# linusmossberg/monte-carlo-ray-tracer

Hardware: NVIDIA H100
Metric: Mray/s (primary+shadow+bounce) (higher is better)
Workload: dtype f64

## Files before the change

### include/mcrt_abi.h

```cpp
#ifndef MCRT_ABI_H
#define MCRT_ABI_H

#include <stddef.h>
#include <stdint.h>

#ifdef __cplusplus
extern "C" {
#endif

#define MCRT_ABI_VERSION 1

typedef enum mcrt_status {
    MCRT_OK = 0,
    MCRT_ERR_INVALID = -1,
    MCRT_ERR_CUDA = -2,
    MCRT_ERR_NO_SCENE = -3,
    MCRT_ERR_UNSUPPORTED = -4,
    MCRT_ERR_NO_PHOTONS = -5
} mcrt_status;

enum { MCRT_PRIM_TRIANGLE = 0, MCRT_PRIM_SPHERE = 1, MCRT_PRIM_QUADRIC = 2 };

enum { MCRT_INTEGRATOR_PATH = 0, MCRT_INTEGRATOR_PHOTON = 1 };

// ... 257 lines not shown
                                    uint32_t tile, const uint8_t* active_tiles, uint32_t sample_first, uint32_t sample_count,
                                    uint32_t global_seed, int integrator_kind, int precision, double* planes_dev,
                                    uint32_t n_planes, mcrt_stats* stats);

enum {
    MCRT_PM_EMISSION = 0, MCRT_PM_DIRECT = 1, MCRT_PM_CAUSTIC = 2, MCRT_PM_GLOBAL = 3, MCRT_PM_COMPONENT_COUNT = 4
};
int mcrt_render_accumulate_photon_components_dev(mcrt_ctx* ctx, const mcrt_camera* camera, uint32_t y_first, uint32_t y_step,
                                                 uint32_t n_rows, uint32_t tile, const uint8_t* active_tiles,
                                                 uint32_t sample_first, uint32_t sample_count, uint32_t global_seed,
                                                 int integrator_kind, int precision, double* planes_dev, uint32_t n_planes,
                                                 mcrt_stats* stats);

enum {
    MCRT_LPE_SYM_RD = 0, MCRT_LPE_SYM_RS = 1, MCRT_LPE_SYM_RG = 2, MCRT_LPE_SYM_TS = 3, MCRT_LPE_SYM_TG = 4,
    MCRT_LPE_SYM_B = 5, MCRT_LPE_SYM_L = 6, MCRT_LPE_SYM_LABEL0 = 7,
    MCRT_LPE_MAX_EXPRESSIONS = 32, MCRT_LPE_MAX_LABELS = 64, MCRT_LPE_MAX_STATES = 255, MCRT_LPE_DEAD = 255,
    MCRT_LPE_MAX_SYMBOLS = MCRT_LPE_SYM_LABEL0 + MCRT_LPE_MAX_LABELS
};
int mcrt_set_light_path_expressions(mcrt_ctx* ctx, const char* const* exprs, uint32_t n);
int mcrt_render_accumulate_lpe_dev(mcrt_ctx* ctx, const mcrt_camera* camera, uint32_t y_first, uint32_t y_step, uint32_t n_rows,
                                   uint32_t tile, const uint8_t* active_tiles, uint32_t sample_first, uint32_t sample_count,
                                   uint32_t global_seed, int integrator_kind, int precision, double* planes_dev,
                                   uint32_t n_planes, mcrt_stats* stats);
int mcrt_lpe_compile_host(const char* const* exprs, uint32_t n, uint32_t n_groups, uint8_t* next, uint32_t* accept,
                          uint8_t* group_symbol, uint32_t* n_states, uint32_t* n_symbols, char* error, uint32_t error_capacity);
int mcrt_lpe_compile_photon_host(const char* const* exprs, uint32_t n, uint32_t n_groups, uint8_t* rev_next, uint32_t* rev_start,
                                 uint32_t* rev_n_states, uint32_t* join, char* error, uint32_t error_capacity);

int mcrt_render_features_dev(mcrt_ctx* ctx, const mcrt_camera* camera, uint32_t sample_first, uint32_t sample_count,
                             uint32_t global_seed, int precision, double* features_dev, mcrt_stats* stats);

#define MCRT_FEATURES_MAX_SPECULAR_DEPTH 7

int mcrt_render_features_chain_dev(mcrt_ctx* ctx, const mcrt_camera* camera, uint32_t sample_first, uint32_t sample_count,
                                   uint32_t global_seed, int precision, uint32_t specular_depth, double* features_dev,
                                   mcrt_stats* stats);

typedef struct mcrt_denoise_params {
    uint32_t iterations;
    uint32_t _pad;
    double sigma_color, sigma_normal, sigma_depth, sigma_albedo;
} mcrt_denoise_params;

#define MCRT_DENOISE_MAX_ITERATIONS 10
#define MCRT_DENOISE_DEFAULT_ITERATIONS 5
#define MCRT_DENOISE_DEFAULT_SIGMA_COLOR 1.0
#define MCRT_DENOISE_DEFAULT_SIGMA_NORMAL 64.0
#define MCRT_DENOISE_DEFAULT_SIGMA_DEPTH 0.1
#define MCRT_DENOISE_DEFAULT_SIGMA_ALBEDO 0.1

int mcrt_denoise_dev(mcrt_ctx* ctx, const double* a_rgb_dev, const double* a_weight_dev,
                     const double* b_rgb_dev, const double* b_weight_dev, const uint32_t* tile_samples,
                     uint32_t tile, const double* features_dev, uint32_t width, uint32_t height,
                     const mcrt_denoise_params* params, double* out_rgb_dev, double* frame_error);

int mcrt_denoise_planes_dev(mcrt_ctx* ctx, const double* a_rgb_dev, const double* b_rgb_dev,
                            const double* a_planes_dev, const double* b_planes_dev, uint32_t n_planes,
                            const uint32_t* tile_samples, uint32_t tile, const double* features_dev,
                            uint32_t width, uint32_t height, const mcrt_denoise_params* params,
                            double* a_out_planes_dev, double* b_out_planes_dev,
                            double* out_rgb_dev, double* frame_error);

int mcrt_frame_alloc(mcrt_ctx* ctx, uint64_t bytes, void** dev_ptr, unsigned char ipc_handle[64]);
int mcrt_frame_open(mcrt_ctx* ctx, const unsigned char ipc_handle[64], void** dev_ptr);
int mcrt_frame_close(mcrt_ctx* ctx, void* peer_ptr);
int mcrt_frame_free(mcrt_ctx* ctx, void* dev_ptr);

int mcrt_bvh4_host(const mcrt_scene_desc* scene, uint32_t max_leaf, void** handle, const void** nodes128, uint32_t* n_nodes);
void mcrt_bvh4_host_free(void* handle);

int mcrt_fp64_peak(mcrt_ctx* ctx, double* dfma_per_second);

int mcrt_trace_closest(mcrt_ctx* ctx, const mcrt_ray* rays, size_t n, int precision,
                       mcrt_hit* hits, mcrt_stats* stats);

int mcrt_sample_rays(mcrt_ctx* ctx, const mcrt_ray* rays, const uint32_t* pixel,
                     const uint32_t* sample, size_t n, uint32_t global_seed,
                     int integrator_kind, int precision, double* out_rgb, mcrt_stats* stats);

int mcrt_sampler_stream(mcrt_ctx* ctx, const uint32_t* pixel, const uint32_t* sample, size_t n,
                        uint32_t n_shuffles, uint32_t global_seed, uint32_t* out_u32x7);

int mcrt_knn_search(mcrt_ctx* ctx, int which, const double* points_xyz, size_t n,
                    uint32_t* out_index, double* out_dist2, uint32_t* out_count,
                    mcrt_stats* stats);

int mcrt_set_option(mcrt_ctx* ctx, const char* key, double value);

#ifdef __cplusplus
}
#endif
#endif
```

### monte-carlo-ray-tracer_b200/__init__.py

```python
import ctypes as C
import math
import os
import struct

import numpy as np

HERE = os.path.dirname(os.path.abspath(__file__))
LIB_PATH = os.environ.get("MCRT_LIB", os.path.join(HERE, "libmcrt_b200.so"))

INTEGRATOR_PATH, INTEGRATOR_PHOTON = 0, 1
PRECISION_F64, PRECISION_F32 = 0, 1
PRIM_TRIANGLE, PRIM_SPHERE, PRIM_QUADRIC = 0, 1, 2
NO_PRIM = 0xFFFFFFFF

ABI_SYMBOLS = [
    "mcrt_abi_version", "mcrt_init", "mcrt_destroy", "mcrt_last_error", "mcrt_scene_upload",
    "mcrt_photon_upload", "mcrt_photon_emit", "mcrt_photon_download", "mcrt_octree_build",
    "mcrt_octree_free", "mcrt_render_rows", "mcrt_render_rows_dev", "mcrt_render_rows_strided_dev",
    "mcrt_trace_closest",
    "mcrt_sample_rays", "mcrt_sampler_stream", "mcrt_knn_search", "mcrt_set_option", "mcrt_set_film",
    "mcrt_obj_load", "mcrt_obj_free", "mcrt_obj_vertex_normals",
    "mcrt_bvh_build", "mcrt_bvh_free", "mcrt_image_tonemap", "mcrt_image_tonemap_dev",
    "mcrt_render_rows_strided_peers", "mcrt_frame_alloc", "mcrt_frame_open", "mcrt_frame_close", "mcrt_frame_free",
    "mcrt_render_film_sums_strided_dev", "mcrt_film_resolve_dev",
    "mcrt_bvh4_host", "mcrt_bvh4_host_free",
    "mcrt_fp64_peak", "mcrt_photon_emit_total", "mcrt_photon_emit_range", "mcrt_photon_build_dev",
    "mcrt_render_accumulate_dev", "mcrt_progressive_resolve_dev",
    "mcrt_render_accumulate_tiles_dev", "mcrt_progressive_resolve_tiles_dev",
    "mcrt_render_features_dev", "mcrt_denoise_dev", "mcrt_render_features_chain_dev",
    "mcrt_photon_emit_pass", "mcrt_photon_gather_radius", "mcrt_photon_gather_search",
    "mcrt_set_light_groups", "mcrt_render_accumulate_groups_dev", "mcrt_light_groups_combine_dev",
    "mcrt_render_accumulate_aovs_dev", "mcrt_photon_download_lights", "mcrt_render_accumulate_photon_components_dev",
    "mcrt_set_light_path_expressions", "mcrt_render_accumulate_lpe_dev", "mcrt_lpe_compile_host",
    "mcrt_lpe_compile_photon_host", "mcrt_photon_download_lpe_states", "mcrt_denoise_planes_dev",
]

AOV_NAMES = ("background", "emission", "diffuse_direct", "diffuse_indirect", "reflection_direct", "reflection_indirect",
             "transmission_direct", "transmission_indirect")

PHOTON_COMPONENT_NAMES = ("emission", "direct", "caustic", "global")

LPE_SYM_RD, LPE_SYM_RS, LPE_SYM_RG, LPE_SYM_TS, LPE_SYM_TG, LPE_SYM_B, LPE_SYM_L, LPE_SYM_LABEL0 = range(8)
LPE_DEAD, LPE_MAX_STATES, LPE_MAX_SYMBOLS, LPE_MAX_EXPRESSIONS = 255, 255, 71, 32
AOV_LPES = ("CB", "CL", "C<RD>[LB]", "C<RD>.+[LB]", "C[<RS><RG>][LB]", "C[<RS><RG>].+[LB]", "C<T.>[LB]", "C<T.>.+[LB]")


def PM_COMPONENT_LPES(direct_visualization):
    n = "[<RD><RG><TG>]"
    if direct_visualization:
        return ("C<.S>*L", "C.*B", f"C<.S>*{n}<.S>.*L", f"C<.S>*{n}({n}.*)?L")
    return ("C<.S>*L", f"C<.S>*{n}L", f"C<.S>*{n}{{1,2}}<.S>.*L", f"C<.S>*{n}{{2}}({n}.*)?L")


class McrtError(RuntimeError):
    pass


class DenoiseParams(C.Structure):
    _fields_ = [("iterations", C.c_uint32), ("_pad", C.c_uint32), ("sigma_color", C.c_double), ("sigma_normal", C.c_double),
                ("sigma_depth", C.c_double), ("sigma_albedo", C.c_double)]


DENOISE_DEFAULTS = {"iterations": 5, "sigma_color": 1.0, "sigma_normal": 64.0, "sigma_depth": 0.1, "sigma_albedo": 0.1}
FEATURES_MAX_SPECULAR_DEPTH = 7


class MaterialRec(C.Structure):
    _fields_ = [("reflectance", C.c_double * 3), ("specular_reflectance", C.c_double * 3),
                ("transmittance", C.c_double * 3), ("emittance", C.c_double * 3),
                ("roughness", C.c_double), ("specular_roughness", C.c_double), ("ior", C.c_double),
                ("transparency", C.c_double), ("complex_ior_real", C.c_double * 3),
                ("complex_ior_imag", C.c_double * 3), ("A", C.c_double), ("B", C.c_double),
                ("a", C.c_double * 2), ("has_complex_ior", C.c_uint32), ("perfect_mirror", C.c_uint32),
                ("rough", C.c_uint32), ("rough_specular", C.c_uint32), ("opaque", C.c_uint32),
                ("emissive", C.c_uint32), ("dirac_delta", C.c_uint32), ("_pad", C.c_uint32)]


MATERIAL_DTYPE = np.dtype([
    ("reflectance", "<f8", 3), ("specular_reflectance", "<f8", 3), ("transmittance", "<f8", 3),
    ("emittance", "<f8", 3), ("roughness", "<f8"), ("specular_roughness", "<f8"), ("ior", "<f8"),
    ("transparency", "<f8"), ("complex_ior_real", "<f8", 3), ("complex_ior_imag", "<f8", 3),
    ("A", "<f8"), ("B", "<f8"), ("a", "<f8", 2), ("has_complex_ior", "<u4"), ("perfect_mirror", "<u4"),
    ("rough", "<u4"), ("rough_specular", "<u4"), ("opaque", "<u4"), ("emissive", "<u4"),
    ("dirac_delta", "<u4"), ("_pad", "<u4")])
assert MATERIAL_DTYPE.itemsize == C.sizeof(MaterialRec)


class SceneDesc(C.Structure):
    _fields_ = [("abi_version", C.c_uint32), ("n_nodes", C.c_uint32),
                ("node_bounds", C.c_void_p), ("node_first_prim", C.c_void_p),
                ("node_prim_count", C.c_void_p), ("node_next_sibling", C.c_void_p),
                ("n_prims", C.c_uint32),
                ("prim_type", C.c_void_p), ("prim_index", C.c_void_p), ("prim_material", C.c_void_p),
                ("prim_area", C.c_void_p),
                ("n_tris", C.c_uint32),
                ("tri_v0", C.c_void_p), ("tri_v1", C.c_void_p), ("tri_v2", C.c_void_p),
                ("tri_e1", C.c_void_p), ("tri_e2", C.c_void_p), ("tri_normal", C.c_void_p),
                ("tri_vn_index", C.c_void_p),
                ("n_vertex_normals", C.c_uint32), ("vertex_normals", C.c_void_p),
                ("n_spheres", C.c_uint32), ("sphere_origin_radius", C.c_void_p),
                ("n_quadrics", C.c_uint32),
                ("quadric_Q", C.c_void_p), ("quadric_G", C.c_void_p), ("quadric_bounds", C.c_void_p),
                ("n_materials", C.c_uint32), ("materials", C.c_void_p),
# ... 91 lines not shown
        L.mcrt_init.argtypes = [C.c_int, C.POINTER(C.c_void_p)]
        L.mcrt_destroy.argtypes = [C.c_void_p]
        L.mcrt_destroy.restype = None
        L.mcrt_last_error.argtypes = [C.c_void_p]
        L.mcrt_last_error.restype = C.c_char_p
        L.mcrt_scene_upload.argtypes = [C.c_void_p, C.POINTER(SceneDesc), C.POINTER(C.c_uint64)]
        L.mcrt_photon_upload.argtypes = [C.c_void_p, C.POINTER(PhotonMapDesc), C.POINTER(PhotonMapDesc),
                                         C.c_uint32, C.c_uint32, C.POINTER(C.c_uint64)]
        L.mcrt_photon_emit.argtypes = [C.c_void_p, C.POINTER(PhotonEmitParams), C.c_int, C.POINTER(C.c_uint64),
                                       C.POINTER(C.c_uint64), C.POINTER(Stats)]
        L.mcrt_photon_emit_pass.argtypes = [C.c_void_p, C.POINTER(PhotonEmitParams), C.c_int, C.c_uint32, C.POINTER(C.c_uint64),
                                            C.POINTER(C.c_uint64), C.POINTER(Stats)]
        L.mcrt_photon_gather_radius.argtypes = [C.c_void_p, C.c_double, C.c_double]
        L.mcrt_photon_gather_search.argtypes = [C.c_void_p, C.c_int, C.c_void_p, C.c_size_t, C.c_double, C.c_void_p, C.c_void_p,
                                                C.c_void_p, C.POINTER(Stats)]
        L.mcrt_photon_download.argtypes = [C.c_void_p, C.c_int, C.POINTER(PhotonMapDesc)]
        L.mcrt_photon_download_lights.argtypes = [C.c_void_p, C.c_int, C.c_void_p, C.c_uint64]
        L.mcrt_photon_download_lpe_states.argtypes = [C.c_void_p, C.c_int, C.c_void_p, C.c_uint64]
        L.mcrt_octree_build.argtypes = [C.c_void_p, C.c_void_p, C.c_uint64, C.c_uint32, C.c_void_p, C.POINTER(C.c_void_p),
                                        C.POINTER(PhotonMapDesc), C.POINTER(C.c_double)]
        L.mcrt_octree_free.argtypes = [C.c_void_p]
        L.mcrt_octree_free.restype = None
        render_args = [C.c_void_p, C.POINTER(CameraRec), C.c_uint32, C.c_uint32, C.c_uint32, C.c_uint32,
                       C.c_int, C.c_int, C.c_void_p, C.POINTER(Stats)]
        L.mcrt_render_rows.argtypes = render_args
        L.mcrt_render_rows_dev.argtypes = render_args
        L.mcrt_render_rows_strided_dev.argtypes = [C.c_void_p, C.POINTER(CameraRec), C.c_uint32, C.c_uint32, C.c_uint32,
                                                   C.c_uint32, C.c_uint32, C.c_int, C.c_int, C.c_void_p, C.POINTER(Stats)]
        L.mcrt_render_rows_strided_peers.argtypes = [C.c_void_p, C.POINTER(CameraRec), C.c_uint32, C.c_uint32, C.c_uint32, C.c_uint32,
                                                     C.c_uint32, C.c_int, C.c_int, C.c_void_p, C.c_uint32, C.c_int, C.POINTER(Stats)]
        L.mcrt_frame_alloc.argtypes = [C.c_void_p, C.c_uint64, C.POINTER(C.c_void_p), C.c_void_p]
        L.mcrt_frame_open.argtypes = [C.c_void_p, C.c_void_p, C.POINTER(C.c_void_p)]
        L.mcrt_frame_close.argtypes = [C.c_void_p, C.c_void_p]
        L.mcrt_frame_free.argtypes = [C.c_void_p, C.c_void_p]
        L.mcrt_fp64_peak.argtypes = [C.c_void_p, C.POINTER(C.c_double)]
        L.mcrt_bvh4_host.argtypes = [C.POINTER(SceneDesc), C.c_uint32, C.POINTER(C.c_void_p), C.POINTER(C.c_void_p), C.POINTER(C.c_uint32)]
        L.mcrt_bvh4_host_free.argtypes = [C.c_void_p]
        L.mcrt_bvh4_host_free.restype = None
        L.mcrt_render_film_sums_strided_dev.argtypes = [C.c_void_p, C.POINTER(CameraRec), C.c_uint32, C.c_uint32, C.c_uint32, C.c_uint32,
                                                        C.c_uint32, C.c_int, C.c_int, C.c_void_p, C.c_void_p, C.POINTER(Stats)]
        L.mcrt_film_resolve_dev.argtypes = [C.c_void_p, C.c_void_p, C.c_void_p, C.c_uint64, C.c_void_p]
        L.mcrt_render_accumulate_dev.argtypes = [C.c_void_p, C.POINTER(CameraRec), C.c_uint32, C.c_uint32, C.c_uint32, C.c_uint32,
                                                 C.c_uint32, C.c_uint32, C.c_int, C.c_int, C.c_void_p, C.c_void_p, C.POINTER(Stats)]
        L.mcrt_progressive_resolve_dev.argtypes = [C.c_void_p, C.c_void_p, C.c_void_p, C.c_uint64, C.c_void_p, C.c_void_p, C.c_uint64,
                                                   C.c_uint32, C.c_uint32, C.c_uint32, C.c_void_p, C.c_void_p, C.POINTER(C.c_double)]
        L.mcrt_render_accumulate_tiles_dev.argtypes = [C.c_void_p, C.POINTER(CameraRec), C.c_uint32, C.c_uint32, C.c_uint32, C.c_uint32,
                                                       C.c_void_p, C.c_uint32, C.c_uint32, C.c_uint32, C.c_int, C.c_int, C.c_void_p,
                                                       C.c_void_p, C.POINTER(Stats)]
        L.mcrt_progressive_resolve_tiles_dev.argtypes = [C.c_void_p, C.c_void_p, C.c_void_p, C.c_void_p, C.c_void_p, C.c_void_p,
                                                         C.c_uint32, C.c_uint32, C.c_uint32, C.c_void_p, C.c_void_p, C.c_void_p,
                                                         C.POINTER(C.c_double)]
        L.mcrt_set_light_groups.argtypes = [C.c_void_p, C.c_void_p, C.c_uint32, C.c_uint32]
        L.mcrt_render_accumulate_groups_dev.argtypes = [C.c_void_p, C.POINTER(CameraRec), C.c_uint32, C.c_uint32, C.c_uint32, C.c_uint32,
                                                        C.c_void_p, C.c_uint32, C.c_uint32, C.c_uint32, C.c_int, C.c_int, C.c_void_p,
                                                        C.c_uint32, C.POINTER(Stats)]
        L.mcrt_render_accumulate_aovs_dev.argtypes = L.mcrt_render_accumulate_groups_dev.argtypes
        L.mcrt_render_accumulate_photon_components_dev.argtypes = L.mcrt_render_accumulate_groups_dev.argtypes
        L.mcrt_set_light_path_expressions.argtypes = [C.c_void_p, C.c_void_p, C.c_uint32]
        L.mcrt_render_accumulate_lpe_dev.argtypes = L.mcrt_render_accumulate_groups_dev.argtypes
        L.mcrt_lpe_compile_host.argtypes = [C.c_void_p, C.c_uint32, C.c_uint32, C.c_void_p, C.c_void_p, C.c_void_p,
                                            C.POINTER(C.c_uint32), C.POINTER(C.c_uint32), C.c_char_p, C.c_uint32]
        L.mcrt_lpe_compile_photon_host.argtypes = [C.c_void_p, C.c_uint32, C.c_uint32, C.c_void_p, C.POINTER(C.c_uint32),
                                                   C.POINTER(C.c_uint32), C.c_void_p, C.c_char_p, C.c_uint32]
        L.mcrt_light_groups_combine_dev.argtypes = [C.c_void_p, C.c_void_p, C.c_uint32, C.c_uint64, C.c_void_p, C.c_void_p]
        L.mcrt_render_features_dev.argtypes = [C.c_void_p, C.POINTER(CameraRec), C.c_uint32, C.c_uint32, C.c_uint32, C.c_int,
                                               C.c_void_p, C.POINTER(Stats)]
        L.mcrt_render_features_chain_dev.argtypes = [C.c_void_p, C.POINTER(CameraRec), C.c_uint32, C.c_uint32, C.c_uint32, C.c_int,
                                                     C.c_uint32, C.c_void_p, C.POINTER(Stats)]
        L.mcrt_denoise_dev.argtypes = [C.c_void_p, C.c_void_p, C.c_void_p, C.c_void_p, C.c_void_p, C.c_void_p, C.c_uint32,
                                       C.c_void_p, C.c_uint32, C.c_uint32, C.POINTER(DenoiseParams), C.c_void_p,
                                       C.POINTER(C.c_double)]
        L.mcrt_denoise_planes_dev.argtypes = [C.c_void_p, C.c_void_p, C.c_void_p, C.c_void_p, C.c_void_p, C.c_uint32, C.c_void_p,
                                              C.c_uint32, C.c_void_p, C.c_uint32, C.c_uint32, C.POINTER(DenoiseParams), C.c_void_p,
                                              C.c_void_p, C.c_void_p, C.POINTER(C.c_double)]
        L.mcrt_photon_emit_total.argtypes = [C.c_void_p, C.POINTER(PhotonEmitParams), C.POINTER(C.c_uint64)]
        L.mcrt_photon_emit_range.argtypes = [C.c_void_p, C.POINTER(PhotonEmitParams), C.c_int, C.c_uint64, C.c_uint64, C.POINTER(C.c_void_p),
                                             C.POINTER(C.c_uint64), C.POINTER(C.c_void_p), C.POINTER(C.c_uint64), C.POINTER(Stats)]
        L.mcrt_photon_build_dev.argtypes = [C.c_void_p, C.POINTER(PhotonEmitParams), C.c_void_p, C.c_uint64, C.c_void_p, C.c_uint64,
                                            C.POINTER(C.c_double)]
        L.mcrt_trace_closest.argtypes = [C.c_void_p, C.c_void_p, C.c_size_t, C.c_int, C.c_void_p, C.POINTER(Stats)]
        L.mcrt_sample_rays.argtypes = [C.c_void_p, C.c_void_p, C.c_void_p, C.c_void_p, C.c_size_t, C.c_uint32,
                                       C.c_int, C.c_int, C.c_void_p, C.POINTER(Stats)]
        L.mcrt_sampler_stream.argtypes = [C.c_void_p, C.c_void_p, C.c_void_p, C.c_size_t, C.c_uint32, C.c_uint32, C.c_void_p]
        L.mcrt_knn_search.argtypes = [C.c_void_p, C.c_int, C.c_void_p, C.c_size_t, C.c_void_p, C.c_void_p,
                                      C.c_void_p, C.POINTER(Stats)]
        L.mcrt_set_option.argtypes = [C.c_void_p, C.c_char_p, C.c_double]
        L.mcrt_set_film.argtypes = [C.c_void_p, C.POINTER(FilmRec)]
        L.mcrt_bvh_build.argtypes = [C.c_void_p, C.c_void_p, C.c_uint32, C.c_void_p, C.c_int, C.c_int,
                                     C.POINTER(C.c_void_p), C.POINTER(BvhDesc), C.POINTER(C.c_double)]
        L.mcrt_bvh_free.argtypes = [C.c_void_p]
        L.mcrt_bvh_free.restype = None
        L.mcrt_obj_load.argtypes = [C.c_char_p, C.c_int, C.POINTER(C.c_void_p), C.POINTER(ObjMeshRec), C.c_char_p, C.c_size_t]
        L.mcrt_obj_free.argtypes = [C.c_void_p]
        L.mcrt_obj_free.restype = None
        L.mcrt_obj_vertex_normals.argtypes = [C.c_void_p, C.c_uint64, C.c_void_p, C.c_uint64, C.c_int, C.c_void_p]
        tm_args = [C.c_void_p, C.c_void_p, C.c_uint32, C.c_uint32, C.POINTER(ImageParams), C.c_void_p,
                   C.POINTER(C.c_double), C.POINTER(C.c_double)]
        L.mcrt_image_tonemap.argtypes = tm_args
        L.mcrt_image_tonemap_dev.argtypes = tm_args
        if L.mcrt_abi_version() != 1:
            raise McrtError("libmcrt_b200.so ABI version mismatch")
        _lib = L
    return _lib


def _ptr(a):
    return a.ctypes.data_as(C.c_void_p) if a is not None and a.size else None


_PACK_DTYPES = {0: np.uint8, 1: np.uint32, 2: np.int32, 3: np.uint64, 4: np.float32, 5: np.float64}


def read_pack(path):
    if path.endswith(".xz"):
        import lzma
        with lzma.open(path, "rb") as f:
            blob = f.read()
    else:
        with open(path, "rb") as f:
            blob = f.read()
    if blob[:8] != b"MCRTPK01":
        raise McrtError(f"{path}: not a scene pack")
    n, = struct.unpack_from("<I", blob, 8)
    out = {}
    for i in range(n):
        name, dtype, elem_size, count, offset = struct.unpack_from("<32sIIQQ", blob, 16 + 56 * i)
        name = name.split(b"\0")[0].decode()
        if dtype == 6:
            if name != "materials" or elem_size != MATERIAL_DTYPE.itemsize:
                raise McrtError(f"{path}: unexpected struct entry {name}")
            arr = np.frombuffer(blob, dtype=MATERIAL_DTYPE, count=count, offset=offset)
        else:
            arr = np.frombuffer(blob, dtype=_PACK_DTYPES[dtype], count=count, offset=offset)
        out[name] = arr.copy()
    return out


class Scene:

    _ARRAYS = ["node_bounds", "node_first_prim", "node_prim_count", "node_next_sibling", "prim_type",
               "prim_index", "prim_material", "prim_area", "tri_v0", "tri_v1", "tri_v2", "tri_e1", "tri_e2",
               "tri_normal", "tri_vn_index", "vertex_normals", "sphere_origin_radius", "quadric_Q",
               "quadric_G", "quadric_bounds", "materials", "light_prim", "light_cdf"]

    def __init__(self, arrays):
        self.a = {k: np.ascontiguousarray(arrays[k]) for k in self._ARRAYS}
        self.ior = float(np.asarray(arrays["scene_ior"]).reshape(-1)[0])
        self.extra = {k: v for k, v in arrays.items() if k not in self._ARRAYS}

    @classmethod
    def from_pack(cls, path):
        return cls(read_pack(path))

    @property
    def n_prims(self):
        return int(self.a["prim_type"].size)

    @property
    def n_nodes(self):
        return int(self.a["node_first_prim"].size)

    @property
    def n_lights(self):
        return int(self.a["light_prim"].size)

    def desc(self):
# ... 358 lines not shown
        return self.last_stats

    def denoise_dev(self, a_rgb_ptr, a_weight_ptr, b_rgb_ptr, b_weight_ptr, tile_samples, tile, features_ptr, width, height,
                    out_ptr, params=None):
        def p(x):
            return C.c_void_p(x) if x else None
        counts = np.ascontiguousarray(tile_samples, dtype=np.uint32)
        if counts.shape != tile_grid(height, width, tile) + (2,):
            raise McrtError(f"tile_samples has shape {counts.shape}, expected {tile_grid(height, width, tile) + (2,)}")
        err = C.c_double()
        self._check(lib().mcrt_denoise_dev(self.ctx, p(a_rgb_ptr), p(a_weight_ptr), p(b_rgb_ptr), p(b_weight_ptr),
                                           counts.ctypes.data_as(C.c_void_p), tile, p(features_ptr), width, height,
                                           C.byref(params) if params is not None else None, p(out_ptr), C.byref(err)))
        return err.value

    def denoise_planes_dev(self, a_rgb_ptr, b_rgb_ptr, a_planes_ptr, b_planes_ptr, n_planes, tile_samples, tile, features_ptr,
                           width, height, a_out_ptr, b_out_ptr, params=None, out_ptr=None):
        def p(x):
            return C.c_void_p(x) if x else None
        counts = np.ascontiguousarray(tile_samples, dtype=np.uint32)
        if counts.shape != tile_grid(height, width, tile) + (2,):
            raise McrtError(f"tile_samples has shape {counts.shape}, expected {tile_grid(height, width, tile) + (2,)}")
        err = C.c_double()
        self._check(lib().mcrt_denoise_planes_dev(self.ctx, p(a_rgb_ptr), p(b_rgb_ptr), p(a_planes_ptr), p(b_planes_ptr), n_planes,
                                                  counts.ctypes.data_as(C.c_void_p), tile, p(features_ptr), width, height,
                                                  C.byref(params) if params is not None else None, p(a_out_ptr), p(b_out_ptr),
                                                  p(out_ptr), C.byref(err) if out_ptr else None))
        return err.value if out_ptr else None

    def frame_alloc(self, nbytes):
        ptr = C.c_void_p(); h = (C.c_ubyte * 64)()
        self._check(lib().mcrt_frame_alloc(self.ctx, nbytes, C.byref(ptr), h))
        return ptr.value, bytes(h)

    def frame_open(self, handle):
        ptr = C.c_void_p(); h = (C.c_ubyte * 64)(*handle)
        self._check(lib().mcrt_frame_open(self.ctx, h, C.byref(ptr)))
        return ptr.value

    def frame_close(self, ptr):
        self._check(lib().mcrt_frame_close(self.ctx, C.c_void_p(ptr)))

    def frame_free(self, ptr):
        self._check(lib().mcrt_frame_free(self.ctx, C.c_void_p(ptr)))

    def fp64_peak(self):
        v = C.c_double()
        self._check(lib().mcrt_fp64_peak(self.ctx, C.byref(v)))
        return v.value

    def render_rows_strided_dev(self, camera, out_dev_ptr, y_first, y_step, n_rows, sqrtspp=None, precision=None):
        self.set_film(camera)
        st = Stats()
        self._check(lib().mcrt_render_rows_strided_dev(self.ctx, C.byref(camera.rec), y_first, y_step, n_rows,
                                                       camera.sqrtspp if sqrtspp is None else sqrtspp,
                                                       self.global_seed, self.kind,
                                                       self.precision if precision is None else precision,
                                                       C.c_void_p(out_dev_ptr), C.byref(st)))
        self.last_stats = st.as_dict()
        return self.last_stats

    def tonemap(self, rgb, image=None):
        params = image if isinstance(image, ImageParams) else ImageParams.from_json(image or {})
        rgb = np.ascontiguousarray(rgb, dtype=np.float64)
        h, w = rgb.shape[:2]
        out = np.zeros((h, w, 3), dtype=np.uint8)
        e, g = C.c_double(), C.c_double()
        self._check(lib().mcrt_image_tonemap(self.ctx, _ptr(rgb), w, h, C.byref(params), _ptr(out), C.byref(e), C.byref(g)))
        return out, e.value, g.value

    def tonemap_dev(self, rgb_dev_ptr, out_dev_ptr, width, height, image=None):
        params = image if isinstance(image, ImageParams) else ImageParams.from_json(image or {})
        e, g = C.c_double(), C.c_double()
        self._check(lib().mcrt_image_tonemap_dev(self.ctx, C.c_void_p(rgb_dev_ptr), width, height, C.byref(params),
                                                 C.c_void_p(out_dev_ptr), C.byref(e), C.byref(g)))
        return e.value, g.value

    def sampler_stream(self, pixel, sample, n_shuffles):
        pixel = np.ascontiguousarray(pixel, dtype=np.uint32)
        sample = np.ascontiguousarray(sample, dtype=np.uint32)
        out = np.zeros((len(pixel), 7), dtype=np.uint32)
        self._check(lib().mcrt_sampler_stream(self.ctx, _ptr(pixel), _ptr(sample), len(pixel), n_shuffles,
                                              self.global_seed, _ptr(out)))
        return out


class PathTracer(Integrator):
    kind = INTEGRATOR_PATH


class PhotonMapper(Integrator):
    kind = INTEGRATOR_PHOTON

    def __init__(self, scene, device=0, precision=PRECISION_F64, global_seed=0x12345678, photon_maps=None, emit=None):
        super().__init__(scene, device, precision, global_seed)
        if emit is not None:
            self.emit(**emit)
            return
        maps = photon_maps or scene.photon_maps()
        if maps is None:
            raise McrtError("PhotonMapper needs photon maps (scene pack exported with photon_map=True) or emit=...")
        self._maps = maps
        self.upload_photons()

    @property
    def has_photon_lights(self):
        return getattr(self, "_photon_lights", False)

    @property
    def has_photon_lpe_states(self):
        key = getattr(self, "_photon_lpe_key", None)
        return key is not None and getattr(self, "_emitted", None) is not None and key == getattr(self, "_lpe_key", None)

    def photon_lpe_states(self, which):
        out = np.zeros(self.n_photons[which], np.uint32)
        self._check(lib().mcrt_photon_download_lpe_states(self.ctx, int(which), _ptr(out), out.size))
        return out

    def emit_again(self):
        if getattr(self, "_emit_args", None) is None:
            raise McrtError("the photon maps did not come from emit() / emit_pass()")
        return self.emit_pass(*self._emit_args)

    def photon_lights(self, which):
        if not self.has_photon_lights:
            raise McrtError("the photon maps carry no light index: only the maps of emit() / emit_pass() do")
        out = np.zeros(self.n_photons[which], np.uint32)
        self._check(lib().mcrt_photon_download_lights(self.ctx, int(which), _ptr(out), out.size))
        return out

    def set_light_groups(self, ids, n_groups=None):
        if not self.has_photon_lights:
            raise McrtError("the photon mapper has no light groups with these maps: their photons carry no light index "
                            "(only the maps of emit() / emit_pass() do)")
        return super().set_light_groups(ids, n_groups)

    def render_accumulate_aovs_dev(self, *args, **kwargs):
        raise McrtError("the photon mapper has no light-path AOVs")

    def render_accumulate_components_dev(self, camera, planes_ptr, sample_first, sample_count, tile=0, active=None,
                                         y_first=0, y_step=1, n_rows=None, precision=None):
        return self._render_accumulate_planes(lib().mcrt_render_accumulate_photon_components_dev, camera, planes_ptr,
                                              len(PHOTON_COMPONENT_NAMES), sample_first, sample_count, tile, active, y_first,
                                              y_step, n_rows, precision)

    def _emit_params(self, emissions, caustic_factor, max_photons_per_octree_leaf, k_nearest_photons, direct_visualization, scene_bounds):
        p = PhotonEmitParams()
        p.emissions = int(emissions); p.caustic_factor = float(caustic_factor)
        p.max_photons_per_octree_leaf = int(max_photons_per_octree_leaf); p.k_nearest_photons = int(k_nearest_photons)
        p.direct_visualization = int(bool(direct_visualization)); p.global_seed = self.global_seed
        if scene_bounds is not None:
            b = scene_bounds
        elif self.scene.a["node_bounds"].size >= 6:
            b = self.scene.a["node_bounds"][:6]
        elif "scene_bounds" in self.scene.extra:
            b = self.scene.extra["scene_bounds"]
        else:
            raise McrtError("the scene has no BVH and no scene bounds: pass scene_bounds")
        for i in range(6):
            p.scene_bounds[i] = float(b[i])
        return p

    def emit_sharded(self, rank, world, emissions, caustic_factor, max_photons_per_octree_leaf=200, k_nearest_photons=50,
                     direct_visualization=False, scene_bounds=None, precision=None):
        import torch
        from . import distributed as mdist
# ... 837 lines not shown
```

### monte-carlo-ray-tracer_b200/csrc/abi.cu

```cuda
#include <algorithm>
#include <cmath>
#include <cstdio>
#include <cstdlib>
#include <cstring>
#include <string>
#include <vector>

#include "mcrt_abi.h"
#include "launch.h"
#include "bvh_build.h"
#include "image.h"
#include "denoise.h"
#include "lpe.h"

using namespace mcrt;

static const int MCRT_INTERNAL_EMIT = 100;

#define CK(call)                                                                              \
    do {                                                                                      \
        cudaError_t e_ = (call);                                                              \
        if (e_ != cudaSuccess)                                                                \
        {                                                                                     \
            ctx->error = std::string(#call) + ": " + cudaGetErrorString(e_);                  \
// ... 472 lines not shown
            const Pending pn = queue[q];
            const uint32_t self = (uint32_t)out.size();
            out.emplace_back();
            out[pn.parent].child[pn.slot] = self;
            expand(pn.item, kids);
            too_big = emit(kids, self) != 0;
        }
        if (too_big) out.clear();
        return MCRT_OK;
    }

    template <class R>
    int uploadArrays(mcrt_ctx* ctx, const mcrt_scene_desc& s, SceneArrays<R>& a, uint64_t& bytes)
    {
        DeviceScene<R>& d = a.dev;
        int rc;
        if ((rc = devUpload(ctx, ctx->scene_allocs, &d.wide, a.wide, bytes))) return rc;
        if ((rc = devUpload(ctx, ctx->scene_allocs, &d.geom, a.geom, bytes))) return rc;
        if ((rc = devUpload(ctx, ctx->scene_allocs, &d.shade, a.shade, bytes))) return rc;
        if ((rc = devUpload(ctx, ctx->scene_allocs, &d.vnormals, a.vnormals, bytes))) return rc;
        if ((rc = devUpload(ctx, ctx->scene_allocs, &d.quadrics, a.quadrics, bytes))) return rc;
        if ((rc = devUpload(ctx, ctx->scene_allocs, &d.materials, a.materials, bytes))) return rc;
        if ((rc = devUpload(ctx, ctx->scene_allocs, &d.lights, a.lights, bytes))) return rc;
        {
            std::vector<uint32_t> combos;
            std::vector<uint8_t> cls(s.n_prims ? s.n_prims : 1, 1);
            for (uint32_t i = 0; i < s.n_prims; i++)
            {
                const uint32_t combo = (a.materials[a.shade[i].material].flags << 1) | (a.shade[i].vn_index >= 0 ? 1u : 0u);
                size_t k = 0;
                while (k < combos.size() && combos[k] != combo) k++;
                if (k == combos.size()) combos.push_back(combo);
                cls[i] = (uint8_t)(1u + (k < SHADE_CLASS_BINS - 1u ? k : SHADE_CLASS_BINS - 2u));
            }
            if ((rc = devUpload(ctx, ctx->scene_allocs, &d.shade_class, cls, bytes))) return rc;
        }
        d.n_nodes = s.n_nodes; d.n_prims = s.n_prims; d.n_lights = s.n_lights;
        d.prims_class = PRIMS_TRI;
        for (uint32_t i = 0; i < s.n_prims; i++)
        {
            if (s.prim_type[i] == MCRT_PRIM_SPHERE && d.prims_class == PRIMS_TRI) d.prims_class = PRIMS_TRI_SPHERE;
            else if (s.prim_type[i] != MCRT_PRIM_TRIANGLE && s.prim_type[i] != MCRT_PRIM_SPHERE) { d.prims_class = PRIMS_ALL; break; }
        }
        d.material_flags_any = 0;
        for (const auto& m : a.materials) d.material_flags_any |= m.flags;
        d.scene_ior = (R)s.scene_ior;
        d.scene_scale = (R)ctx->scene_scale;
        return MCRT_OK;
    }

    template <class R>
    int ensureWave(mcrt_ctx* ctx, WaveBuffers<R>& w, std::vector<void*>& track)
    {
        if (w.capacity == ctx->pool_paths) return MCRT_OK;
        freeAll(track);
        w.capacity = 0;
        const size_t n = ctx->pool_paths;
        int rc;
        for (int b = 0; b < 2; b++)
        {
            if ((rc = devAlloc(ctx, track, &w.buf[b].ray_o, n))) return rc;
            if ((rc = devAlloc(ctx, track, &w.buf[b].ray_d, n))) return rc;
            if ((rc = devAlloc(ctx, track, &w.buf[b].thr, n))) return rc;
            if ((rc = devAlloc(ctx, track, &w.buf[b].iors_a, n))) return rc;
            if ((rc = devAlloc(ctx, track, &w.buf[b].iors_b, n))) return rc;
            if ((rc = devAlloc(ctx, track, &w.buf[b].meta, n))) return rc;
            if ((rc = devAlloc(ctx, track, &w.buf[b].meta2, n))) return rc;
        }
        if ((rc = devAlloc(ctx, track, &w.shadow, n))) return rc;
        if ((rc = devAlloc(ctx, track, &w.hits, n))) return rc;
        w.capacity = ctx->pool_paths;
        return MCRT_OK;
    }

    int ensureSort(mcrt_ctx* ctx)
    {
        if (ctx->sort_capacity == ctx->pool_paths) return MCRT_OK;
        freeAll(ctx->sort_allocs);
        ctx->sort_capacity = 0;
        const size_t n = ctx->pool_paths;
        int rc;
        RaySort& r = ctx->sort;
        for (int b = 0; b < 2; b++)
        {
            if ((rc = devAlloc(ctx, ctx->sort_allocs, &r.path_key[b], n))) return rc;
            if ((rc = devAlloc(ctx, ctx->sort_allocs, &r.path_rank[b], n))) return rc;
        }
        if ((rc = devAlloc(ctx, ctx->sort_allocs, &r.path_order, n))) return rc;
        if ((rc = devAlloc(ctx, ctx->sort_allocs, &r.shadow_key, n))) return rc;
        if ((rc = devAlloc(ctx, ctx->sort_allocs, &r.shadow_rank, n))) return rc;
        if ((rc = devAlloc(ctx, ctx->sort_allocs, &r.shadow_order, n))) return rc;
        if ((rc = devAlloc(ctx, ctx->sort_allocs, &r.shade_key, n))) return rc;
        if ((rc = devAlloc(ctx, ctx->sort_allocs, &r.shade_rank, n))) return rc;
        if ((rc = devAlloc(ctx, ctx->sort_allocs, &r.shade_order, n))) return rc;
        if ((rc = devAlloc(ctx, ctx->sort_allocs, &r.hist_shade, (size_t)SORT_BINS))) return rc;
        if ((rc = devAlloc(ctx, ctx->sort_allocs, &r.hist_path, (size_t)SORT_BINS))) return rc;
        if ((rc = devAlloc(ctx, ctx->sort_allocs, &r.hist_shadow, (size_t)SORT_BINS))) return rc;
        if ((rc = devAlloc(ctx, ctx->sort_allocs, &r.bin_start, (size_t)SORT_BINS))) return rc;
        if ((rc = devAlloc(ctx, ctx->sort_allocs, &r.block_offset, (size_t)2 * SORT_SCAN_BLOCKS))) return rc;
        if ((rc = devAlloc(ctx, ctx->sort_allocs, &r.done_counter, (size_t)1))) return rc;
        CK(cudaMemset(r.done_counter, 0, sizeof(uint32_t)));
        ctx->sort_capacity = ctx->pool_paths;
        return MCRT_OK;
    }

    int ensureFilm(mcrt_ctx* ctx, size_t values)
    {
        if (ctx->film_values >= values && ctx->d_film) return MCRT_OK;
        if (ctx->d_film) cudaFree(ctx->d_film);
        ctx->d_film = nullptr; ctx->film_values = 0;
        CK(cudaMalloc((void**)&ctx->d_film, values * sizeof(double)));
        ctx->film_values = values;
        return MCRT_OK;
    }

    template <class R> DeviceScene<R>& sceneOf(mcrt_ctx* ctx);
    template <> DeviceScene<double>& sceneOf<double>(mcrt_ctx* ctx) { return ctx->scene64; }
    template <> DeviceScene<float>& sceneOf<float>(mcrt_ctx* ctx) { return ctx->scene32; }
    template <class R> WaveBuffers<R>& waveOf(mcrt_ctx* ctx);
    template <> WaveBuffers<double>& waveOf<double>(mcrt_ctx* ctx) { return ctx->wave64; }
    template <> WaveBuffers<float>& waveOf<float>(mcrt_ctx* ctx) { return ctx->wave32; }
    template <class R> std::vector<void*>& waveAllocsOf(mcrt_ctx* ctx);
    template <> std::vector<void*>& waveAllocsOf<double>(mcrt_ctx* ctx) { return ctx->wave_allocs64; }
    template <> std::vector<void*>& waveAllocsOf<float>(mcrt_ctx* ctx) { return ctx->wave_allocs32; }

    void fillStats(mcrt_stats* st, const Counters& c, uint64_t iterations, uint64_t launches, double ms)
    {
        if (!st) return;
        std::memset(st, 0, sizeof(*st));
        st->paths = c.paths;
        st->extension_rays = c.extension_rays;
        st->shadow_rays = c.shadow_rays;
        st->box_tests = c.box_tests;
        st->prim_tests = c.prim_tests;
        st->knn_queries = c.knn_queries;
        st->wavefront_iterations = iterations;
        st->kernel_launches = launches;
        st->ior_stack_overflows = c.ior_stack_overflows;
        st->max_depth = c.max_depth;
        st->gpu_ms_total = ms;
        st->shadow_box_tests = c.shadow_box_tests;
        st->shadow_prim_tests = c.shadow_prim_tests;
        st->extend_work_sum = c.work_sum;
        st->extend_work_warpmax = c.work_warpmax;
        st->replayed_rays = c.replayed_rays;
    }

    template <class R> DeviceCamera<R> deviceCamera(const mcrt_camera& cam)
    {
        DeviceCamera<R> c;
        std::memset(&c, 0, sizeof(c));
        c.eye = v3<R>(cam.eye); c.forward = v3<R>(cam.forward);
        c.left = v3<R>(cam.left); c.up = v3<R>(cam.up);
        c.focal_length = (R)cam.focal_length; c.sensor_width = (R)cam.sensor_width;
        c.aperture_radius = (R)cam.aperture_radius; c.focus_distance = (R)cam.focus_distance;
        c.width = cam.width; c.height = cam.height; c.thin_lens = cam.thin_lens;
        return c;
    }

    template <class R> R rayEps(const mcrt_ctx* ctx)
    {
        return Mode<R>::parity ? (R)1e-9 : (R)(ctx->ray_eps_scale * ctx->scene_scale);
    }

    struct FilmSums
    {
        double* rgb;
        double* wsum;
        uint32_t n_planes = 0;
        bool aovs = false;
        bool lpe = false;
    };

    template <class R>
    int runWavefront(mcrt_ctx* ctx, const mcrt_camera* cam, uint32_t row_first, uint32_t row_step, uint32_t n_pixels, uint32_t spp,
                     uint64_t total_work, uint32_t global_seed, int integrator, const double* d_user_rays,
                     const uint32_t* d_user_pixel, const uint32_t* d_user_sample, size_t film_pixels,
                     double film_weight, double* out_dev, mcrt_stats* stats, uint32_t sample_first = 0,
                     const FilmSums* accum = nullptr, const uint32_t* d_pixel_list = nullptr)
    {
        if (!ctx->has_scene) { ctx->error = "no scene uploaded"; return MCRT_ERR_NO_SCENE; }
        if (integrator == MCRT_INTEGRATOR_PHOTON && !ctx->has_photons)
        {
// ... 83 lines not shown
        if (ctx->sort_rays)
        {
            if ((rc = ensureSort(ctx))) return rc;
            p.sort = ctx->sort;
            p.sort.shade_sorted = ctx->sort_shade ? 1u : 0u;
            if (!ctx->sort_shade_class || integrator == MCRT_INTERNAL_EMIT) p.sort.shade_order = nullptr;
            {
                const uint32_t n_prims = sceneOf<R>(ctx).n_prims;
                const double cells = (double)(1u << (3 * SORT_ORIGIN_BITS));
                const bool use_prim = (ctx->sort_prim_key < 0 ? n_prims >= 4096u : ctx->sort_prim_key != 0) && (double)n_prims >= cells;
                p.sort.prim_scale = use_prim ? (uint32_t)(cells * 4294967296.0 / (double)n_prims * 0.999999) : 0u;
            }
            for (int k = 0; k < 3; k++)
            {
                const double ext = ctx->scene_bmax[k] - ctx->scene_bmin[k];
                p.sort.key_min[k] = (float)ctx->scene_bmin[k];
                p.sort.key_scale[k] = ext > 0.0 ? (float)((double)(1u << SORT_ORIGIN_BITS) / ext) : 0.0f;
            }
        }

        const bool emitting = integrator == MCRT_INTERNAL_EMIT;
        if (emitting)
        {
            p.emit.emit_offsets = ctx->d_emit_offsets;
            p.emit.photon_flux = static_cast<const V4<R>*>(ctx->d_emit_flux);
            p.emit.photons[0] = ctx->d_emit_photons[0]; p.emit.photons[1] = ctx->d_emit_photons[1];
            p.emit.lights[0] = ctx->d_emit_lights[0]; p.emit.lights[1] = ctx->d_emit_lights[1];
            p.emit.capacity[0] = ctx->emit_capacity[0]; p.emit.capacity[1] = ctx->emit_capacity[1];
            p.emit.non_caustic_reject = (R)ctx->emit_non_caustic_reject;
            p.emit.pass = ctx->emit_pass;
            if (ctx->d_emit_lpe_states[0])
            {
                p.emit.lpe_states[0] = ctx->d_emit_lpe_states[0]; p.emit.lpe_states[1] = ctx->d_emit_lpe_states[1];
                p.emit.lpe_rev_next = ctx->d_lpe_rev_next;
                p.emit.lpe_rev_start = ctx->lpe_rev_start;
                p.lpe_light_symbol = ctx->d_lpe_light_symbol;
                p.lpe_symbols = ctx->lpe_symbols;
            }
        }
        if (integrator == MCRT_INTEGRATOR_PHOTON)
        {
            p.pm.map[0] = ctx->photon_map[0]; p.pm.map[1] = ctx->photon_map[1];
            p.pm.queries = knn_queue;
            p.pm.k_nearest = ctx->k_nearest;
            p.pm.direct_visualization = ctx->direct_visualization;
            p.pm.query_capacity = knn_capacity;
            p.pm.gather_r2[0] = ctx->gather_r2[0]; p.pm.gather_r2[1] = ctx->gather_r2[1];
            if (ctx->photon_lights) { p.pm.lights[0] = ctx->built_dev[0].lights; p.pm.lights[1] = ctx->built_dev[1].lights; }
            if (accum && accum->lpe)
            {
                p.pm.lpe_states[0] = ctx->built_dev[0].lpe_states; p.pm.lpe_states[1] = ctx->built_dev[1].lpe_states;
                p.pm.lpe_join = ctx->d_lpe_join;
                p.pm.lpe_join_any = ctx->d_lpe_join_any;
                p.pm.lpe_rev_states = ctx->lpe_rev_states;
            }
        }

        Counters init;
        std::memset(&init, 0, sizeof(init));
        init.total_work = total_work;
        if (sample_first)
        {
            init.next_work = (uint64_t)sample_first * n_pixels;
            init.total_work = init.next_work + total_work;
        }
        if (integrator == MCRT_INTERNAL_EMIT) { init.next_work = ctx->emit_work_first; init.total_work = ctx->emit_work_first + total_work; }
        ctx->h_counters[0] = init;
        CK(cudaEventRecord(ctx->ev_start, s));
        CK(cudaMemcpyAsync(ctx->d_counters, &ctx->h_counters[0], sizeof(Counters), cudaMemcpyHostToDevice, s));
        if (!accum)
        {
            CK(cudaMemsetAsync(ctx->d_film, 0, film_pixels * 3 * sizeof(double), s));
            if (filtered) CK(cudaMemsetAsync(ctx->d_film_wsum, 0, film_pixels * sizeof(double), s));
        }
        const bool sorting = ctx->sort_rays != 0;
        if (sorting)
        {
            CK(cudaMemsetAsync(p.sort.hist_path, 0, SORT_BINS * sizeof(uint32_t), s));
            CK(cudaMemsetAsync(p.sort.hist_shadow, 0, SORT_BINS * sizeof(uint32_t), s));
            CK(cudaMemsetAsync(ctx->sort.hist_shade, 0, SORT_BINS * sizeof(uint32_t), s));
        }
        auto sortPaths = [&](int buffer)
        {
            launchSortScan(p.sort.hist_path, p.sort, s);
            launchSortScatter(p.sort.path_key[buffer], p.sort.path_rank[buffer], p.sort, p.sort.path_order,
                              &ctx->d_counters->n_cur, grid, s);
        };

        uint64_t launches = 0, iterations = 0;

        if (emitting) Launch<R>::emitGenerate(p, 0, grid, s);
        else Launch<R>::generate(p, 0, grid, s);
        launchAdvance(ctx->d_counters, s);
        launches += 2;
        if (sorting) { sortPaths(0); launches += 2; }

        int pending[2] = { 0, 0 };
        int slot = 0;
        bool done = false;
        while (!done)
        {
            for (int k = 0; k < ctx->poll_interval; k++)
            {
                const int cur = (int)(iterations & 1u);
                cudaEvent_t* ev = nullptr;
                if (ctx->stage_timing)
                {
                    while (ctx->stage_events.size() < 6 * (iterations + 1))
                    {
                        cudaEvent_t e;
                        CK(cudaEventCreate(&e));
                        ctx->stage_events.push_back(e);
                    }
                    ev = &ctx->stage_events[6 * iterations];
                    cudaEventRecord(ev[0], s);
                }
                Launch<R>::extend(p, cur, grid, s);
                if (ev) cudaEventRecord(ev[1], s);
                if (p.sort.shade_order)
                {
                    Launch<R>::shadeKey(p, grid, s);
                    launchSortScan(p.sort.hist_shade, p.sort, s);
                    launchSortScatter(p.sort.shade_key, p.sort.shade_rank, p.sort, p.sort.shade_order, &ctx->d_counters->n_cur, grid, s);
                    launches += 3;
                }
                if (emitting)
                {
                    Launch<R>::emitShade(p, cur, grid, s);
                }
                else if (integrator == MCRT_INTEGRATOR_PHOTON)
                {
                    Launch<R>::shadePhoton(p, cur, grid, s);
                    if (ev) cudaEventRecord(ev[5], s);
                    Launch<R>::knn(p, grid, s);
                    launches += 1;
                }
                else
                {
                    Launch<R>::shade(p, cur, grid, s);
                }
                if (ev) cudaEventRecord(ev[2], s);
                if (!emitting)
                {
                    if (sorting)
                    {
                        launchSortScan(p.sort.hist_shadow, p.sort, s);
                        launchSortScatter(p.sort.shadow_key, p.sort.shadow_rank, p.sort, p.sort.shadow_order,
                                          &ctx->d_counters->n_shadow, grid, s);
                        launches += 2;
                    }
                    Launch<R>::shadow(p, grid, s);
                }
                if (ev) cudaEventRecord(ev[3], s);
                if (emitting) Launch<R>::emitGenerate(p, cur ^ 1, grid, s);
                else Launch<R>::generate(p, cur ^ 1, grid, s);
                launchAdvance(ctx->d_counters, s);
                if (sorting) { sortPaths(cur ^ 1); launches += 2; }
                if (ev) cudaEventRecord(ev[4], s);
                launches += 5;
                iterations++;
            }
            CK(cudaMemcpyAsync(&ctx->h_counters[slot], ctx->d_counters, sizeof(Counters), cudaMemcpyDeviceToHost, s));
            CK(cudaEventRecord(ctx->ev_poll[slot], s));
            pending[slot] = 1;
            const int other = slot ^ 1;
            if (pending[other])
            {
                CK(cudaEventSynchronize(ctx->ev_poll[other]));
                const Counters& c = ctx->h_counters[other];
                if (c.n_cur == 0 && c.next_work >= c.total_work) done = true;
                pending[other] = 0;
            }
            slot = other;
        }

        if (!emitting && !accum)
        {
            if (filtered) launchResolveFilmWeighted(ctx->d_film, ctx->d_film_wsum, out_dev, film_pixels, grid, s);
            else if (ctx->peer_out.n_frames) launchResolveFilmPeers(ctx->d_film, ctx->peer_out, film_pixels * 3, film_weight, grid, s);
            else launchResolveFilm(ctx->d_film, out_dev, film_pixels * 3, film_weight, grid, s);
            launches += 1;
        }
        CK(cudaEventRecord(ctx->ev_stop, s));
        CK(cudaMemcpyAsync(&ctx->h_counters[0], ctx->d_counters, sizeof(Counters), cudaMemcpyDeviceToHost, s));
        CK(cudaStreamSynchronize(s));
        CK(cudaGetLastError());
        float ms = 0.f;
        CK(cudaEventElapsedTime(&ms, ctx->ev_start, ctx->ev_stop));
        const Counters& c = ctx->h_counters[0];
        fillStats(stats, c, iterations, launches, ms);
        if (stats)
        {
            stats->extend_launches = iterations;
            stats->shadow_launches = iterations;
            if (ctx->stage_timing)
            {
                for (uint64_t it = 0; it < iterations; it++)
                {
                    cudaEvent_t* ev = &ctx->stage_events[6 * it];
                    if (integrator == MCRT_INTEGRATOR_PHOTON) { float tk = 0; cudaEventElapsedTime(&tk, ev[5], ev[2]); stats->gpu_ms_knn += tk; }
                    float t01 = 0, t12 = 0, t23 = 0, t34 = 0;
                    cudaEventElapsedTime(&t01, ev[0], ev[1]); cudaEventElapsedTime(&t12, ev[1], ev[2]);
                    cudaEventElapsedTime(&t23, ev[2], ev[3]); cudaEventElapsedTime(&t34, ev[3], ev[4]);
                    stats->gpu_ms_extend += t01; stats->gpu_ms_shade += t12;
                    stats->gpu_ms_shadow += t23; stats->gpu_ms_generate += t34;
                }
            }
        }
        if (c.traversal_overflow)
        {
            ctx->error = "traversal stack/heap overflow: result would differ from the reference";
            return MCRT_ERR_UNSUPPORTED;
        }
        if (c.ior_stack_overflows)
        {
            ctx->error = "more than 8 nested dielectric media on a path (refraction-history stack overflow): result would differ from the reference";
            return MCRT_ERR_UNSUPPORTED;
        }
        if (emitting && c.photon_overflow)
        {
            ctx->error = "photon arrays overflowed";
            return MCRT_ERR_UNSUPPORTED;
        }
        return MCRT_OK;
    }

    int renderDispatch(mcrt_ctx* ctx, const mcrt_camera* camera, uint32_t y_first, uint32_t y_step, uint32_t n_rows,
                       uint32_t sample_first, uint64_t spp, uint32_t global_seed, int integrator_kind, int precision,
                       double* out_dev, mcrt_stats* stats, const FilmSums* accum = nullptr,
                       const uint32_t* d_pixel_list = nullptr, uint32_t n_list = 0)
    {
        if (!camera || n_rows == 0 || y_step == 0 || spp == 0 || camera->width == 0 ||
            (uint64_t)y_first + (uint64_t)(n_rows - 1) * y_step >= camera->height)
        {
            ctx->error = "mcrt_render_rows: invalid camera / row range / sample count";
            return MCRT_ERR_INVALID;
        }
        if ((uint64_t)sample_first + spp > 0x100000000ull)
        {
            ctx->error = "sample range beyond 2^32 samples per pixel";
// ... 1641 lines not shown
        rc = runWavefront<float>(ctx, nullptr, 0, 1, 0, 1, n, global_seed, integrator_kind, d_rays, d_pixel, d_sample, n, 1.0, d_out, stats);
    else { ctx->error = "unknown precision"; rc = MCRT_ERR_INVALID; }
    if (rc == MCRT_OK && cudaMemcpy(out_rgb, d_out, n * 3 * sizeof(double), cudaMemcpyDeviceToHost) != cudaSuccess)
    { ctx->error = "copy back failed"; rc = MCRT_ERR_CUDA; }
    cleanup();
    return rc;
}

int mcrt_trace_closest(mcrt_ctx* ctx, const mcrt_ray* rays, size_t n, int precision, mcrt_hit* hits, mcrt_stats* stats)
{
    if (!ctx) return MCRT_ERR_INVALID;
    if (n == 0) return MCRT_OK;
    if (!rays || !hits) { ctx->error = "mcrt_trace_closest: null buffer"; return MCRT_ERR_INVALID; }
    if (!ctx->has_scene) { ctx->error = "no scene uploaded"; return MCRT_ERR_NO_SCENE; }
    CK(cudaSetDevice(ctx->device));
    double* d_rays = nullptr; double* d_tuv = nullptr; uint32_t* d_prim = nullptr;
    auto cleanup = [&]() { cudaFree(d_rays); cudaFree(d_tuv); cudaFree(d_prim); };
    if (cudaMalloc((void**)&d_rays, n * 6 * sizeof(double)) != cudaSuccess || cudaMalloc((void**)&d_tuv, n * 3 * sizeof(double)) != cudaSuccess ||
        cudaMalloc((void**)&d_prim, n * 4) != cudaSuccess)
    { cleanup(); ctx->error = "cudaMalloc failed"; return MCRT_ERR_CUDA; }
    cudaStream_t s = ctx->stream;
    cudaMemcpyAsync(d_rays, rays, n * 6 * sizeof(double), cudaMemcpyHostToDevice, s);
    cudaMemsetAsync(ctx->d_counters, 0, sizeof(Counters), s);
    const int grid = ctx->sm_count * ctx->blocks_per_sm;
    cudaEventRecord(ctx->ev_start, s);
    if (precision == MCRT_PRECISION_F64)
    {
        DeviceScene<double> sc = ctx->scene64;
        if (ctx->exact_traversal) sc.bvh4 = nullptr;
        Launch<double>::traceUser(sc, d_rays, n, d_tuv, d_prim, ctx->d_counters, grid, s);
    }
    else if (precision == MCRT_PRECISION_F32) Launch<float>::traceUser(ctx->scene32, d_rays, n, d_tuv, d_prim, ctx->d_counters, grid, s);
    else { cleanup(); ctx->error = "unknown precision"; return MCRT_ERR_INVALID; }
    cudaEventRecord(ctx->ev_stop, s);
    std::vector<double> tuv(n * 3);
    std::vector<uint32_t> prim(n);
    cudaMemcpyAsync(tuv.data(), d_tuv, n * 3 * sizeof(double), cudaMemcpyDeviceToHost, s);
    cudaMemcpyAsync(prim.data(), d_prim, n * 4, cudaMemcpyDeviceToHost, s);
    cudaMemcpyAsync(&ctx->h_counters[0], ctx->d_counters, sizeof(Counters), cudaMemcpyDeviceToHost, s);
    cudaError_t e = cudaStreamSynchronize(s);
    if (e == cudaSuccess) e = cudaGetLastError();
    cleanup();
    if (e != cudaSuccess) { ctx->error = cudaGetErrorString(e); return MCRT_ERR_CUDA; }
    float ms = 0.f;
    cudaEventElapsedTime(&ms, ctx->ev_start, ctx->ev_stop);
    fillStats(stats, ctx->h_counters[0], 0, 1, ms);
    for (size_t i = 0; i < n; i++)
    {
        const bool interp = prim[i] != NO_PRIM && ctx->prim_interpolates[prim[i]];
        hits[i].t = tuv[3 * i];
        hits[i].u = interp ? tuv[3 * i + 1] : 0.0;
        hits[i].v = interp ? tuv[3 * i + 2] : 0.0;
        hits[i].prim = prim[i];
        hits[i].interpolate = interp ? 1u : 0u;
    }
    if (ctx->h_counters[0].traversal_overflow) { ctx->error = "traversal stack/heap overflow"; return MCRT_ERR_UNSUPPORTED; }
    return MCRT_OK;
}

int mcrt_sampler_stream(mcrt_ctx* ctx, const uint32_t* pixel, const uint32_t* sample, size_t n, uint32_t n_shuffles,
                        uint32_t global_seed, uint32_t* out_u32x7)
{
    if (!ctx) return MCRT_ERR_INVALID;
    if (n == 0) return MCRT_OK;
    if (!pixel || !sample || !out_u32x7) { ctx->error = "mcrt_sampler_stream: null buffer"; return MCRT_ERR_INVALID; }
    CK(cudaSetDevice(ctx->device));
    uint32_t* d_pixel = nullptr; uint32_t* d_sample = nullptr; uint32_t* d_out = nullptr;
    auto cleanup = [&]() { cudaFree(d_pixel); cudaFree(d_sample); cudaFree(d_out); };
    if (cudaMalloc((void**)&d_pixel, n * 4) != cudaSuccess || cudaMalloc((void**)&d_sample, n * 4) != cudaSuccess ||
        cudaMalloc((void**)&d_out, n * 28) != cudaSuccess)
    { cleanup(); ctx->error = "cudaMalloc failed"; return MCRT_ERR_CUDA; }
    cudaStream_t s = ctx->stream;
    cudaMemcpyAsync(d_pixel, pixel, n * 4, cudaMemcpyHostToDevice, s);
    cudaMemcpyAsync(d_sample, sample, n * 4, cudaMemcpyHostToDevice, s);
    launchSamplerStream(d_pixel, d_sample, n, n_shuffles, global_seed, d_out, s);
    cudaMemcpyAsync(out_u32x7, d_out, n * 28, cudaMemcpyDeviceToHost, s);
    cudaError_t e = cudaStreamSynchronize(s);
    if (e == cudaSuccess) e = cudaGetLastError();
    cleanup();
    if (e != cudaSuccess) { ctx->error = cudaGetErrorString(e); return MCRT_ERR_CUDA; }
    return MCRT_OK;
}

int mcrt_knn_search(mcrt_ctx* ctx, int which, const double* points_xyz, size_t n, uint32_t* out_index, double* out_dist2,
                    uint32_t* out_count, mcrt_stats* stats)
{
    if (!ctx) return MCRT_ERR_INVALID;
    if (n == 0) return MCRT_OK;
    if (!points_xyz || !out_index || !out_dist2 || !out_count || (which != 0 && which != 1))
    { ctx->error = "mcrt_knn_search: invalid arguments"; return MCRT_ERR_INVALID; }
    if (!ctx->has_photons) { ctx->error = "no photon maps uploaded"; return MCRT_ERR_NO_PHOTONS; }
    CK(cudaSetDevice(ctx->device));
    const uint32_t k = ctx->k_nearest;
    double* d_pts = nullptr; uint32_t* d_idx = nullptr; double* d_d2 = nullptr; uint32_t* d_cnt = nullptr; uint32_t* d_flag = nullptr;
    auto cleanup = [&]() { cudaFree(d_pts); cudaFree(d_idx); cudaFree(d_d2); cudaFree(d_cnt); cudaFree(d_flag); };
    if (cudaMalloc((void**)&d_pts, n * 24) != cudaSuccess || cudaMalloc((void**)&d_idx, n * k * 4) != cudaSuccess ||
        cudaMalloc((void**)&d_d2, n * k * 8) != cudaSuccess || cudaMalloc((void**)&d_cnt, n * 4) != cudaSuccess ||
        cudaMalloc((void**)&d_flag, 4) != cudaSuccess)
    { cleanup(); ctx->error = "cudaMalloc failed"; return MCRT_ERR_CUDA; }
    cudaStream_t s = ctx->stream;
    cudaMemcpyAsync(d_pts, points_xyz, n * 24, cudaMemcpyHostToDevice, s);
    cudaMemsetAsync(d_flag, 0, 4, s);
    cudaEventRecord(ctx->ev_start, s);
    launchKnnUser(ctx->photon_map[which], k, d_pts, n, d_idx, d_d2, d_cnt, d_flag, ctx->sm_count * ctx->blocks_per_sm, s);
    cudaEventRecord(ctx->ev_stop, s);
    uint32_t flag = 0;
    cudaMemcpyAsync(out_index, d_idx, n * k * 4, cudaMemcpyDeviceToHost, s);
    cudaMemcpyAsync(out_dist2, d_d2, n * k * 8, cudaMemcpyDeviceToHost, s);
    cudaMemcpyAsync(out_count, d_cnt, n * 4, cudaMemcpyDeviceToHost, s);
    cudaMemcpyAsync(&flag, d_flag, 4, cudaMemcpyDeviceToHost, s);
    cudaError_t e = cudaStreamSynchronize(s);
    if (e == cudaSuccess) e = cudaGetLastError();
    cleanup();
    if (e != cudaSuccess) { ctx->error = cudaGetErrorString(e); return MCRT_ERR_CUDA; }
    float ms = 0.f;
    cudaEventElapsedTime(&ms, ctx->ev_start, ctx->ev_stop);
    if (stats) { std::memset(stats, 0, sizeof(*stats)); stats->knn_queries = n; stats->gpu_ms_total = ms; stats->gpu_ms_knn = ms; }
    if (flag) { ctx->error = "k-NN frontier overflow"; return MCRT_ERR_UNSUPPORTED; }
    return MCRT_OK;
}

int mcrt_photon_gather_radius(mcrt_ctx* ctx, double r_caustic, double r_global)
{
    if (!ctx) return MCRT_ERR_INVALID;
    if (r_caustic == 0.0 && r_global == 0.0) { ctx->gather_r2[0] = ctx->gather_r2[1] = 0.0; return MCRT_OK; }
    const double r[2] = { r_caustic, r_global };
    for (int w = 0; w < 2; w++)
        if (!(r[w] > 0.0) || !std::isfinite(r[w] * r[w]))
        { ctx->error = "mcrt_photon_gather_radius: radii must be (0, 0) or two positive finite numbers"; return MCRT_ERR_INVALID; }
    ctx->gather_r2[0] = r_caustic * r_caustic; ctx->gather_r2[1] = r_global * r_global;
    return MCRT_OK;
}

int mcrt_photon_gather_search(mcrt_ctx* ctx, int which, const double* points_xyz, size_t n, double radius, uint32_t* out_count,
                              double* out_flux_sum, double* out_cone_sum, mcrt_stats* stats)
{
    if (!ctx) return MCRT_ERR_INVALID;
    if ((which != 0 && which != 1) || !(radius > 0.0) || !std::isfinite(radius * radius))
    { ctx->error = "mcrt_photon_gather_search: invalid arguments"; return MCRT_ERR_INVALID; }
    if (n == 0) return MCRT_OK;
    if (!points_xyz || !out_count || !out_flux_sum || !out_cone_sum) { ctx->error = "mcrt_photon_gather_search: null buffer"; return MCRT_ERR_INVALID; }
    if (!ctx->has_photons) { ctx->error = "no photon maps uploaded"; return MCRT_ERR_NO_PHOTONS; }
    CK(cudaSetDevice(ctx->device));
    double* d_pts = nullptr; uint32_t* d_cnt = nullptr; double* d_flux = nullptr; double* d_cone = nullptr; uint32_t* d_flag = nullptr;
    auto cleanup = [&]() { cudaFree(d_pts); cudaFree(d_cnt); cudaFree(d_flux); cudaFree(d_cone); cudaFree(d_flag); };
    if (cudaMalloc((void**)&d_pts, n * 24) != cudaSuccess || cudaMalloc((void**)&d_cnt, n * 4) != cudaSuccess ||
        cudaMalloc((void**)&d_flux, n * 24) != cudaSuccess || cudaMalloc((void**)&d_cone, n * 24) != cudaSuccess ||
        cudaMalloc((void**)&d_flag, 4) != cudaSuccess)
    { cleanup(); ctx->error = "cudaMalloc failed"; return MCRT_ERR_CUDA; }
    cudaStream_t s = ctx->stream;
    cudaMemcpyAsync(d_pts, points_xyz, n * 24, cudaMemcpyHostToDevice, s);
    cudaMemsetAsync(d_flag, 0, 4, s);
    cudaEventRecord(ctx->ev_start, s);
    launchGatherUser(ctx->photon_map[which], d_pts, n, radius * radius, d_cnt, d_flux, d_cone, d_flag, ctx->sm_count * ctx->blocks_per_sm, s);
    cudaEventRecord(ctx->ev_stop, s);
    uint32_t flag = 0;
    cudaMemcpyAsync(out_count, d_cnt, n * 4, cudaMemcpyDeviceToHost, s);
    cudaMemcpyAsync(out_flux_sum, d_flux, n * 24, cudaMemcpyDeviceToHost, s);
    cudaMemcpyAsync(out_cone_sum, d_cone, n * 24, cudaMemcpyDeviceToHost, s);
    cudaMemcpyAsync(&flag, d_flag, 4, cudaMemcpyDeviceToHost, s);
    cudaError_t e = cudaStreamSynchronize(s);
    if (e == cudaSuccess) e = cudaGetLastError();
    cleanup();
    if (e != cudaSuccess) { ctx->error = cudaGetErrorString(e); return MCRT_ERR_CUDA; }
    float ms = 0.f;
    cudaEventElapsedTime(&ms, ctx->ev_start, ctx->ev_stop);
// ... 7 lines not shown
```

### monte-carlo-ray-tracer_b200/csrc/integrator.cuh

```cuda
#pragma once

#include "bsdf.cuh"
#include "intersect.cuh"
#include "bvh4.cuh"
#include "photon.cuh"
#include "film.cuh"
#include "mcrt_abi.h"

#ifndef MCRT_TRACE_MINBLOCKS_F64
#define MCRT_TRACE_MINBLOCKS_F64 2
#endif
#ifndef MCRT_TRACE_MINBLOCKS_F32
#define MCRT_TRACE_MINBLOCKS_F32 4
#endif
#ifndef MCRT_TRACE_MINBLOCKS_F64_PRUNED
#define MCRT_TRACE_MINBLOCKS_F64_PRUNED 4
#endif
#ifndef MCRT_TRACE_MINBLOCKS_FAST
#define MCRT_TRACE_MINBLOCKS_FAST 2
#endif
#ifndef MCRT_TRACE_MINBLOCKS_DYN
#define MCRT_TRACE_MINBLOCKS_DYN 4
#endif
#ifndef MCRT_KNN_MINBLOCKS
#define MCRT_KNN_MINBLOCKS 8
#endif
#ifndef MCRT_GATHER_MINBLOCKS
#define MCRT_GATHER_MINBLOCKS 3
#endif
#ifndef MCRT_SHADE_MINBLOCKS
#define MCRT_SHADE_MINBLOCKS 3
#endif
#ifndef MCRT_SHADE_MINBLOCKS_LITE
#define MCRT_SHADE_MINBLOCKS_LITE 3
#endif
#ifndef MCRT_SORT_ORIGIN_BITS
#define MCRT_SORT_ORIGIN_BITS 4
#endif
#ifndef MCRT_SORT_DIR_Q
#define MCRT_SORT_DIR_Q 1
#endif

namespace mcrt
{
    constexpr int IOR_STACK_CAPACITY = 8;

    struct Counters
    {
        uint32_t n_cur, n_next, n_shadow, n_gen;
        unsigned long long next_work, total_work;
        unsigned long long paths, extension_rays, shadow_rays, box_tests, prim_tests, knn_queries;
        unsigned long long shadow_box_tests, shadow_prim_tests;
        unsigned long long ior_stack_overflows;
        unsigned long long replayed_rays;
        uint32_t fetch_extend, fetch_shadow;
        uint32_t traversal_overflow, max_depth;
        uint32_t n_knn, _pad;
        unsigned long long work_sum, work_warpmax;
        unsigned long long n_photons[2];
        uint32_t photon_overflow, _pad2;
    };

    template <class R> struct PathBuffer
    {
        V4<R>* ray_o;
        V4<R>* ray_d;
        V4<R>* thr;
        V4<R>* iors_a;
        V4<R>* iors_b;
        uint4* meta;
        uint4* meta2;
    };

    template <class R> struct alignas(16 * sizeof(R)) ShadowRecord
    {
        V4<R> o;
        V4<R> d;
        uint4 meta;
        V4<R> k;
    };
    static_assert(sizeof(ShadowRecord<double>) == 128 && sizeof(ShadowRecord<float>) == 64, "one shadow record per line");
    static_assert(offsetof(ShadowRecord<double>, k) == 96, "the float64 padding is the 16-byte chunk 5 (k_shade writes it)");

    constexpr uint32_t SORT_ORIGIN_BITS = MCRT_SORT_ORIGIN_BITS;
    constexpr uint32_t SORT_DIR_Q = MCRT_SORT_DIR_Q;
    constexpr uint32_t SORT_DIR_BITS = 3 + 2 * SORT_DIR_Q;
    constexpr uint32_t SORT_KEY_BITS = 3 * SORT_ORIGIN_BITS + SORT_DIR_BITS;
    constexpr uint32_t SORT_BINS = 1u << SORT_KEY_BITS;

    struct RaySort
    {
        uint32_t* path_key[2];
        uint32_t* path_rank[2];
        uint32_t* path_order;
        uint32_t* shadow_key;
        uint32_t* shadow_rank;
        uint32_t* shadow_order;
        uint32_t* hist_path;
        uint32_t* hist_shadow;
        uint32_t* bin_start;
        uint32_t* block_offset;
        uint32_t* done_counter;
        uint32_t shade_sorted;
        uint32_t* shade_key;
        uint32_t* shade_rank;
        uint32_t* shade_order;
        uint32_t* hist_shade;
        uint32_t prim_scale;
        float key_min[3], key_scale[3];
    };

    MCRT_D uint32_t spreadBits3(uint32_t v)
    {
        v = (v | (v << 16)) & 0x030000FFu;
        v = (v | (v << 8)) & 0x0300F00Fu;
        v = (v | (v << 4)) & 0x030C30C3u;
        v = (v | (v << 2)) & 0x09249249u;
        return v;
    }

    template <class R>
    MCRT_D uint32_t rayKey(const RaySort& rs, const V3<R>& o, const V3<R>& d, uint32_t src_prim)
    {
        uint32_t cell;
        if (rs.prim_scale && src_prim != NO_PRIM)
        {
            cell = (uint32_t)(((unsigned long long)src_prim * rs.prim_scale) >> 32);
        }
        else
        {
            constexpr float CELLS = (float)(1u << SORT_ORIGIN_BITS);
            float cx = ((float)o.x - rs.key_min[0]) * rs.key_scale[0];
            float cy = ((float)o.y - rs.key_min[1]) * rs.key_scale[1];
            float cz = ((float)o.z - rs.key_min[2]) * rs.key_scale[2];
            uint32_t ix = (uint32_t)fminf(fmaxf(cx, 0.0f), CELLS - 1.0f);
            uint32_t iy = (uint32_t)fminf(fmaxf(cy, 0.0f), CELLS - 1.0f);
            uint32_t iz = (uint32_t)fminf(fmaxf(cz, 0.0f), CELLS - 1.0f);
            cell = spreadBits3(ix) | (spreadBits3(iy) << 1) | (spreadBits3(iz) << 2);
        }
        float dx = (float)d.x, dy = (float)d.y, dz = (float)d.z;
        float ax = fabsf(dx), ay = fabsf(dy), az = fabsf(dz);
        uint32_t face; float u, v, m;
        if (ax >= ay && ax >= az) { face = dx < 0.0f ? 1u : 0u; u = dy; v = dz; m = ax; }
        else if (ay >= az)        { face = dy < 0.0f ? 3u : 2u; u = dx; v = dz; m = ay; }
        else                      { face = dz < 0.0f ? 5u : 4u; u = dx; v = dy; m = az; }
        constexpr float Q = (float)(1u << SORT_DIR_Q);
        float inv = m > 0.0f ? 0.5f * Q / m : 0.0f;
        uint32_t qu = (uint32_t)fminf(fmaxf(u * inv + 0.5f * Q, 0.0f), Q - 1.0f);
        uint32_t qv = (uint32_t)fminf(fmaxf(v * inv + 0.5f * Q, 0.0f), Q - 1.0f);
        uint32_t dir = (face << (2 * SORT_DIR_Q)) | (qu << SORT_DIR_Q) | qv;
        return (dir << (3 * SORT_ORIGIN_BITS)) | cell;
    }

    MCRT_D uint32_t sortRank(uint32_t* hist, uint32_t key, bool pred)
    {
        const unsigned active = __ballot_sync(0xFFFFFFFFu, pred);
        uint32_t rank = 0;
        if (pred)
        {
            const unsigned peers = __match_any_sync(active, key);
            const unsigned lane = threadIdx.x & 31u;
            const int leader = __ffs(peers) - 1;
            uint32_t base = 0;
            if ((int)lane == leader) base = atomicAdd(&hist[key], (uint32_t)__popc(peers));
            base = __shfl_sync(peers, base, leader);
            rank = base + __popc(peers & ((1u << lane) - 1u));
        }
        return rank;
    }

    template <class R> struct EmitParams
    {
        const unsigned long long* emit_offsets;
        const V4<R>* photon_flux;
        float4* photons[2];
        uint32_t* lights[2];
        unsigned long long capacity[2];
        R non_caustic_reject;
        uint32_t pass;
        const uint8_t* lpe_rev_next;
        uint32_t lpe_rev_start;
        uint32_t* lpe_states[2];
    };

    template <class R> struct WaveParams
    {
        DeviceScene<R> scene;
        DeviceCamera<R> camera;
        PathBuffer<R> buf[2];
        ShadowRecord<R>* shadow;
        V4<R>* hits;
        Counters* counters;
        double* film;
        const double* user_rays;
        const uint32_t* user_pixel;
        const uint32_t* user_sample;
        const uint32_t* pixel_list;
        uint32_t capacity;
        uint32_t global_seed;
        uint32_t spp;
        uint32_t row_first;
        uint32_t row_step;
        uint32_t n_pixels;
        uint32_t integrator;
        R ray_eps;
        PhotonParams<R> pm;
        RaySort sort;
        const uint32_t* sobol_bytes;
        EmitParams<R> emit;
        FilmParams filmp;
        const uint32_t* group_of_light;
        size_t plane_values;
        uint32_t n_planes;
        uint32_t aovs;
        const uint8_t* lpe_next;
        const uint32_t* lpe_accept;
        const uint8_t* lpe_light_symbol;
        uint32_t lpe_symbols;
    };

    template <class R> struct Mode;
    template <> struct Mode<double> { static constexpr bool parity = true; static constexpr int trace_minblocks = MCRT_TRACE_MINBLOCKS_F64; static constexpr int trace_minblocks_pruned = MCRT_TRACE_MINBLOCKS_F64_PRUNED; };
    template <> struct Mode<float> { static constexpr bool parity = false; static constexpr int trace_minblocks = MCRT_TRACE_MINBLOCKS_F32; static constexpr int trace_minblocks_pruned = MCRT_TRACE_MINBLOCKS_F32; };

    template <int PRIMS = PRIMS_ALL, bool FAST = false, class R>
    MCRT_D Hit<R> traceClosest(const DeviceScene<R>& sc, const V3<R>& o, const V3<R>& d, uint32_t skip_prim,
                               TraceCounters& cnt, uint32_t& overflow)
    {
        RayQ<R> rq;
        rq.o = o; rq.d = d;
        if constexpr (!(Mode<R>::parity && FAST) || PRIMS == PRIMS_ALL) rq.inv_d = R(1) / d;
        if constexpr (Mode<R>::parity)
        {
            if constexpr (FAST)
            {
                bool ambiguous;
                Hit<R> h = traverseFast<PRIMS>(sc, rq, cnt, ambiguous);
                if (ambiguous)
                {
                    const DeviceScene<R> sc_copy = sc;
                    RayQ<R> rq_copy = rq;
                    rq_copy.inv_d = R(1) / d;
                    Hit<R> h2;
                    traceReferenceOrderOutOfLine<PRIMS>(&sc_copy, &rq_copy, &h2, &cnt.box_tests, &cnt.prim_tests, &overflow);
                    h = h2;
                    cnt.replayed++;
                }
                return h;
            }
            else
            {
// ... 144 lines not shown

    template <class R>
    MCRT_D void cameraRay(const DeviceCamera<R>& c, R scene_ior, uint32_t pixel, const SamplerState& smp,
                          V3<R>& start, V3<R>& direction)
    {
        const uint32_t x = pixel % c.width, y = pixel / c.width;
        R pixel_size = c.sensor_width / R(c.width);
        R half_w = R(c.width) * R(0.5), half_h = R(c.height) * R(0.5);
        R u[2];
        samplerGet<R, DIM_PIXEL, 2>(smp, u);
        R px = R(x) + u[0], py = R(y) + u[1];
        R lx = pixel_size * (half_w - px), ly = pixel_size * (half_h - py);
        direction = normalize(c.forward * c.focal_length + c.left * lx + c.up * ly);
        start = c.eye;
        if (c.thin_lens)
        {
            R ul[2];
            samplerGet<R, DIM_LENS, 2>(smp, ul);
            R azimuth = ul[1] * Consts<R>::TWO_PI;
            R sn, cs;
            msincos(azimuth, &sn, &cs);
            R su = msqrt(ul[0]);
            R ax = (cs * su) * c.aperture_radius, ay = (sn * su) * c.aperture_radius;
            V3<R> focus_point = start + direction * (c.focus_distance / dot(direction, c.forward));
            V3<R> s2 = c.eye + c.left * ax + c.up * ay;
            direction = normalize(focus_point - s2);
            start = s2;
        }
    }

    template <class R, bool FILM, bool LIST>
    __global__ void __launch_bounds__(256) k_generate(WaveParams<R> p, int next)
    {
        Counters* c = p.counters;
        const uint32_t n_next = c->n_next;
        const unsigned long long remaining = c->total_work - c->next_work;
        const uint32_t room = p.capacity - n_next;
        const uint32_t count = remaining < (unsigned long long)room ? (uint32_t)remaining : room;
        if (blockIdx.x == 0 && threadIdx.x == 0) c->n_gen = count;
        const unsigned long long base_work = c->next_work;
        const PathBuffer<R>& out = p.buf[next];

        const uint32_t count_rounded = (count + 31u) & ~31u;
        for (uint32_t j = blockIdx.x * blockDim.x + threadIdx.x; j < count_rounded; j += gridDim.x * blockDim.x)
        {
            const bool valid = j < count;
            uint32_t key = 0;
            const uint32_t slot = n_next + j;
            if (valid)
            {
            const unsigned long long w = base_work + j;
            uint32_t pixel, sample, film_index;
            V3<R> start, direction;
            if (p.user_rays)
            {
                pixel = p.user_pixel[w];
                sample = p.user_sample[w];
                film_index = (uint32_t)w;
                const double* r = p.user_rays + 6 * w;
                start = V3<R>((R)r[0], (R)r[1], (R)r[2]);
                direction = V3<R>((R)r[3], (R)r[4], (R)r[5]);
            }
            else
            {
                uint32_t local = (uint32_t)(w % p.n_pixels);
                if constexpr (LIST) local = p.pixel_list[local];
                sample = (uint32_t)(w / p.n_pixels);
                const uint32_t row = local / p.camera.width, col = local - row * p.camera.width;
                pixel = (p.row_first + row * p.row_step) * p.camera.width + col;
                film_index = local;
                SamplerState smp = SamplerState::make(p.global_seed, pixel, sample, 0u);
                cameraRay(p.camera, p.scene.scene_ior, pixel, smp, start, direction);
                if constexpr (FILM) filmSplatSampleWeight(p.filmp, p.global_seed, pixel, sample);
            }
            stStream(&out.ray_o[slot], V4<R>(start, p.scene.scene_ior));
            stStream(&out.ray_d[slot], V4<R>(direction, R(1)));
            stStream(&out.thr[slot], V4<R>(R(1), R(1), R(1), R(0)));
            stStream(&out.meta[slot], make_uint4(pixel, sample, 0u, 0u));
            stStream(&out.meta2[slot], make_uint4(NO_PRIM, 1u, film_index, NO_PRIM));
            if (p.sort.path_order) key = rayKey(p.sort, start, direction, NO_PRIM);
            }
            if (p.sort.path_order)
            {
                const uint32_t rank = sortRank(p.sort.hist_path, key, valid);
                if (valid) { p.sort.path_key[next][slot] = key; p.sort.path_rank[next][slot] = rank; }
            }
        }
    }

    static __global__ void k_advance(Counters* c)
    {
        c->n_cur = c->n_next + c->n_gen;
        c->next_work += c->n_gen;
        c->paths += c->n_gen;
        c->n_next = 0;
        c->n_gen = 0;
        c->n_shadow = 0;
        c->n_knn = 0;
        c->fetch_extend = 0;
        c->fetch_shadow = 0;
    }

    template <class R, int PRIMS, int FAST>
    __global__ void __launch_bounds__(256, FAST == 2 ? MCRT_TRACE_MINBLOCKS_DYN : (FAST == 1 ? MCRT_TRACE_MINBLOCKS_FAST : (PRIMS == PRIMS_ALL ? Mode<R>::trace_minblocks : Mode<R>::trace_minblocks_pruned))) k_extend(WaveParams<R> p, int cur)
    {
        const uint32_t n = p.counters->n_cur;
        const PathBuffer<R>& in = p.buf[cur];
        TraceCounters cnt = { 0u, 0u, 0u };
        uint32_t overflow = 0;
        unsigned long long rays = 0;
        const uint32_t* order = p.sort.path_order;
        if constexpr (Mode<R>::parity && FAST == 2)
        {
            traceManyFast<PRIMS>(p.scene, n, &p.counters->fetch_extend,
                [&](uint32_t ii, RayQ<R>& r)
                {
                    const uint32_t i = order ? order[ii] : ii;
                    const V4<R> ro = ldStream(&in.ray_o[i]), rd = ldStream(&in.ray_d[i]);
                    r.o = ro.xyz(); r.d = rd.xyz();
                    if constexpr (PRIMS == PRIMS_ALL) r.inv_d = R(1) / r.d;
                    return i;
                },
                [&](uint32_t i, const RayQ<R>&, const Hit<R>& h)
                {
                    stStream(&p.hits[i], V4<R>(h.t, h.u, h.v, h.prim == NO_PRIM ? R(-1) : R(h.prim)));
                    rays++;
                }, cnt, overflow);
            flushStats(p.counters, cnt, rays, false, overflow);
            return;
        }
        for (uint32_t ii = blockIdx.x * blockDim.x + threadIdx.x; ii < n; ii += gridDim.x * blockDim.x)
        {
            const uint32_t i = order ? order[ii] : ii;
            const V4<R> ro = ldStream(&in.ray_o[i]);
            const V4<R> rd = ldStream(&in.ray_d[i]);
            uint32_t skip = NO_PRIM;
            if constexpr (!Mode<R>::parity) skip = in.meta2[i].w;
#ifdef MCRT_TAIL_DIAGNOSTIC
            const uint32_t w0 = cnt.box_tests + cnt.prim_tests;
#endif
            Hit<R> h = traceClosest<PRIMS, FAST != 0>(p.scene, ro.xyz(), rd.xyz(), skip, cnt, overflow);
            stStream(&p.hits[i], V4<R>(h.t, h.u, h.v, h.prim == NO_PRIM ? R(-1) : R(h.prim)));
            rays++;
#ifdef MCRT_TAIL_DIAGNOSTIC
            const uint32_t w = cnt.box_tests + cnt.prim_tests - w0;
            const unsigned am = __activemask();
            const uint32_t wmax = __reduce_max_sync(am, w);
            atomicAdd(&p.counters->work_sum, (unsigned long long)w);
            if ((threadIdx.x & 31u) == (unsigned)(__ffs(am) - 1)) atomicAdd(&p.counters->work_warpmax, 32ull * wmax);
#endif
        }
        flushStats(p.counters, cnt, rays, false, overflow);
    }

    template <class R>
    MCRT_D void sampleLightPoint(const Light<R>& l, R u, R v, V3<R>& pos, V3<R>& normal)
    {
        if (l.type == PRIM_TRIANGLE)
        {
            R su = msqrt(u);
            pos = (R(1) - su) * l.p0 + (R(1) - v) * su * l.p1 + v * su * l.p2;
            normal = l.normal;
        }
        else
        {
            R z = R(1) - R(2) * u;
            R r = msqrt(R(1) - pow2(z));
            R phi = Consts<R>::TWO_PI * v;
// ... 219 lines not shown
                        R cos_light_theta = dot(-s_dir, light_normal);
                        if (cos_light_theta > R(0))
                        {
                            bool ok = true;
                            R cos_theta = dot(s_dir, ia.normal);
                            if (cos_theta <= R(0))
                            {
                                if ((m.flags & MAT_OPAQUE) || cos_theta == R(0)) ok = false;
                                else
                                {
                                    s_start = ia.position - ia.normal * p.ray_eps;
                                    s_dir = normalize(light_pos - s_start);
                                }
                            }
                            if (ok)
                            {
                                V3<R> bsdf_absIdotN; R bsdf_pdf;
                                if (ia.bsdfWorld(bsdf_absIdotN, s_dir, bsdf_pdf))
                                {
                                    want_shadow = true;
                                    sh_o = s_start; sh_d = s_dir;
                                    sh_k = bsdf_absIdotN * L.emittance * throughput;
                                    sh_bsdf_pdf = bsdf_pdf;
                                    sh_area_cos = L.area * cos_light_theta;
                                    sh_select = ls_select;
                                    sh_light = L.prim;
                                    if constexpr (FILM == FILM_MODE_AOV) sh_plane = KIND == 0 ? aovPlane(lobe, ray.depth > 0u, false) : (uint32_t)MCRT_PM_DIRECT;
                                    if constexpr (FILM == FILM_MODE_LPE)
                                    {
                                        sh_plane = lpeAccept(p, lpeNext(p, lpe_state, lpeLightSymbol(p, ls_light)));
                                        want_shadow = sh_plane != 0u;
                                    }
                                }
                            }
                        }
                    }

                    V3<R> bsdf_absIdotN;
                    if (!do_bsdf)
                    {
                    }
                    else if (!sampleBSDF(ia, ray, smp, p.ray_eps, false, bsdf_absIdotN, ls_bsdf_pdf, nray))
                    {
                        alive = false;
                    }
                    else
                    {
                        throughput *= bsdf_absIdotN / ls_bsdf_pdf;
                        R survive = compMax(throughput) * nray.refraction_scale;
                        if (survive == R(0))
                        {
                            alive = false;
                        }
                        else if (nray.diffuse_depth > 3u || nray.depth > 16u)
                        {
                            survive = gmin(R(0.95), survive);
                            R ua;
                            samplerGet<R, DIM_ABSORB, 1>(smp, &ua);
                            if (survive <= ua) alive = false;
                            else throughput /= survive;
                        }
                    }

                    if (alive)
                    {
                        if (nray.refraction_level > 0)
                        {
                            if (nray.refraction_level == (int32_t)ior_count)
                            {
                                if (ior_count < (uint32_t)IOR_STACK_CAPACITY) iors[ior_count++] = nray.medium_ior;
                                else stack_overflows++;
                            }
                            else if (nray.refraction_level < (int32_t)ior_count - 1)
                            {
                                ior_count--;
                            }
                        }
                    }
                }
            }

            const uint32_t slot = warpAppend(&c->n_next, alive);
            const uint32_t sslot = warpAppend(&c->n_shadow, want_shadow);
            uint32_t pkey = 0, prank = 0, skey = 0, srank = 0;
            if (sorting && alive)
            {
                pkey = rayKey(p.sort, nray.start, nray.direction, hit_prim);
                prank = atomicAdd(&p.sort.hist_path[pkey], 1u);
            }
            if (sorting && want_shadow)
            {
                skey = rayKey(p.sort, sh_o, sh_d, hit_prim);
                srank = atomicAdd(&p.sort.hist_shadow[skey], 1u);
            }
            if (alive)
            {
                stStream(&out.ray_o[slot], V4<R>(nray.start, nray.medium_ior));
                stStream(&out.ray_d[slot], V4<R>(nray.direction, nray.refraction_scale));
                stStream(&out.thr[slot], V4<R>(throughput, ls_bsdf_pdf));
                if (ior_count > 1)
                {
                    out.iors_a[slot] = V4<R>(iors[1], iors[2], iors[3], iors[4]);
                    if (ior_count > 5) out.iors_b[slot] = V4<R>(iors[5], iors[6], iors[7], R(0));
                }
                stStream(&out.meta[slot], make_uint4(meta.x, meta.y, (nray.depth & 0xFFFFu) | (nray.diffuse_depth << 16),
                                                     (uint32_t)nray.refraction_level));
                stStream(&out.meta2[slot], make_uint4(ls_light, ior_count | (nray.dirac_delta ? 256u : 0u) | (lobe << 9) |
                                                                    (FILM == FILM_MODE_LPE ? lpe_state << 16 : 0u), meta2.z,
                                                      sc.shade[hit_prim].type == PRIM_TRIANGLE ? hit_prim : NO_PRIM));
                if (sorting) { p.sort.path_key[cur ^ 1][slot] = pkey; p.sort.path_rank[cur ^ 1][slot] = prank; }
            }
            if (want_shadow)
            {
                ShadowRecord<R>& srec = p.shadow[sslot];
                stStream(&srec.o, V4<R>(sh_o, sh_bsdf_pdf));
                stStream(&srec.d, V4<R>(sh_d, sh_area_cos));
                stStream(&srec.meta, make_uint4(sh_light, meta2.z, sc.shade[hit_prim].type == PRIM_TRIANGLE ? hit_prim : NO_PRIM,
                                                FILM == FILM_MODE_AOV || FILM == FILM_MODE_LPE ? sh_plane : meta.y));
                if constexpr (sizeof(R) == 8) stStream(reinterpret_cast<uint4*>(&srec) + 5, make_uint4(0u, 0u, 0u, 0u));
                stStream(&srec.k, V4<R>(sh_k, sh_select));
                if (sorting) { p.sort.shadow_key[sslot] = skey; p.sort.shadow_rank[sslot] = srank; }
            }

            if constexpr (KIND == 1)
            {
                const uint32_t q0 = warpAppend(&c->n_knn, want_knn >= 1);
                if (want_knn >= 1 && q0 < p.pm.query_capacity) p.pm.queries[q0] = knn_q;
                const uint32_t q1 = warpAppend(&c->n_knn, want_knn == 2);
                if (want_knn == 2 && q1 < p.pm.query_capacity)
                {
                    knn_q.meta.z |= 2u;
                    p.pm.queries[q1] = knn_q;
                }
            }
        }

        if (local_max_depth) atomicMax(&c->max_depth, local_max_depth);
        if (stack_overflows) atomicAdd(&c->ior_stack_overflows, (unsigned long long)stack_overflows);
    }

    template <class R, int FILM, int PRIMS, int FAST>
    __global__ void __launch_bounds__(256, FAST == 2 ? MCRT_TRACE_MINBLOCKS_DYN : (FAST == 1 ? MCRT_TRACE_MINBLOCKS_FAST : (PRIMS == PRIMS_ALL ? Mode<R>::trace_minblocks : Mode<R>::trace_minblocks_pruned))) k_shadow(WaveParams<R> p)
    {
        const uint32_t n = p.counters->n_shadow;
        TraceCounters cnt = { 0u, 0u, 0u };
        uint32_t overflow = 0;
        unsigned long long rays = 0;
        const uint32_t* order = p.sort.shadow_order;
        if constexpr (Mode<R>::parity && FAST == 2)
        {
            traceManyFast<PRIMS, true>(p.scene, n, &p.counters->fetch_shadow,
                [&](uint32_t ii, RayQ<R>& r, uint32_t& target)
                {
                    const uint32_t i = order ? order[ii] : ii;
                    const V4<R> so = ldStream(&p.shadow[i].o), sd = ldStream(&p.shadow[i].d);
                    r.o = so.xyz(); r.d = sd.xyz();
                    if constexpr (PRIMS == PRIMS_ALL) r.inv_d = R(1) / r.d;
                    target = p.shadow[i].meta.x;
                    return i;
                },
                [&](uint32_t i, const RayQ<R>&, const Hit<R>& h)
                {
                    rays++;
                    const ShadowRecord<R>& srec = p.shadow[i];
                    const uint4 sm = srec.meta;
                    if (h.prim == sm.x)
                    {
                        const V4<R> so = srec.o, sd = srec.d, sk = srec.k;
                        R light_pdf = pow2(h.t) / sd.w;
                        R mis_weight = powerHeuristic(light_pdf, so.w);
                        depositRadiance<FILM>(p, sm.y, pixelOfFilmIndex(p, sm.y), sm.w, sk.xyz() * (mis_weight / (light_pdf * sk.w)),
                                              FILM == FILM_MODE_GROUPS ? p.scene.shade[sm.x].light : NO_PRIM, sm.w);
                    }
                }, cnt, overflow);
            flushStats(p.counters, cnt, rays, true, overflow);
            return;
        }
        for (uint32_t ii = blockIdx.x * blockDim.x + threadIdx.x; ii < n; ii += gridDim.x * blockDim.x)
        {
            const uint32_t i = order ? order[ii] : ii;
            const ShadowRecord<R>& srec = p.shadow[i];
            const V4<R> so = ldStream(&srec.o), sd = ldStream(&srec.d);
            const uint4 sm = ldStream(&srec.meta);
            Hit<R> h;
            if constexpr (Mode<R>::parity && FAST != 0) h = traceVisible<PRIMS>(p.scene, so.xyz(), sd.xyz(), sm.x, cnt, overflow);
            else h = traceClosest<PRIMS, false>(p.scene, so.xyz(), sd.xyz(), sm.z, cnt, overflow);
            rays++;
            if (h.prim == sm.x)
            {
                const V4<R> sk = srec.k;
                R light_pdf = pow2(h.t) / sd.w;
                R mis_weight = powerHeuristic(light_pdf, so.w);
                depositRadiance<FILM>(p, sm.y, pixelOfFilmIndex(p, sm.y), sm.w, sk.xyz() * (mis_weight / (light_pdf * sk.w)),
                                      FILM == FILM_MODE_GROUPS ? p.scene.shade[sm.x].light : NO_PRIM, sm.w);
            }
        }
        flushStats(p.counters, cnt, rays, true, overflow);
    }



    constexpr uint32_t SHADE_CLASS_BINS = 64;

    template <class R>
    __global__ void __launch_bounds__(256) k_shade_key(WaveParams<R> p)
    {
        __shared__ uint32_t s_hist[SHADE_CLASS_BINS], s_base[SHADE_CLASS_BINS];
        const uint32_t n = p.counters->n_cur;
        const uint32_t chunks = (n + 255u) / 256u;
        for (uint32_t chunk = blockIdx.x; chunk < chunks; chunk += gridDim.x)
        {
            if (threadIdx.x < SHADE_CLASS_BINS) s_hist[threadIdx.x] = 0u;
            __syncthreads();
            const uint32_t i = chunk * 256u + threadIdx.x;
            uint32_t key = 0, local = 0;
            if (i < n)
            {
                const R w = p.hits[i].w;
                if (!(w < R(0))) key = p.scene.shade_class[(uint32_t)w];
                local = atomicAdd(&s_hist[key], 1u);
            }
            __syncthreads();
            if (threadIdx.x < SHADE_CLASS_BINS && s_hist[threadIdx.x]) s_base[threadIdx.x] = atomicAdd(&p.sort.hist_shade[threadIdx.x], s_hist[threadIdx.x]);
            __syncthreads();
            if (i < n) { p.sort.shade_key[i] = key; p.sort.shade_rank[i] = s_base[key] + local; }
            __syncthreads();
        }
    }

    constexpr uint32_t SORT_SCAN_BLOCKS = SORT_BINS / 1024;

    static __global__ void __launch_bounds__(256) k_sort_scan(uint32_t* hist, uint32_t* bin_start, uint32_t* block_offset,
                                                              uint32_t* done_counter)
    {
        __shared__ uint32_t warp_sums[8];
        __shared__ uint32_t is_last;
        const uint32_t t = threadIdx.x, base = blockIdx.x * 1024u + t * 4u;
        const uint4 v = *reinterpret_cast<const uint4*>(hist + base);
        *reinterpret_cast<uint4*>(hist + base) = make_uint4(0u, 0u, 0u, 0u);
        const uint32_t sum = v.x + v.y + v.z + v.w;
        uint32_t incl = sum;
        for (int off = 1; off < 32; off <<= 1)
        {
            const uint32_t u = __shfl_up_sync(0xFFFFFFFFu, incl, off);
            if ((t & 31u) >= (uint32_t)off) incl += u;
        }
        if ((t & 31u) == 31u) warp_sums[t >> 5] = incl;
        __syncthreads();
        uint32_t warp_base = 0;
        for (uint32_t w = 0; w < (t >> 5); w++) warp_base += warp_sums[w];
        const uint32_t excl = warp_base + incl - sum;
        *reinterpret_cast<uint4*>(bin_start + base) = make_uint4(excl, excl + v.x, excl + v.x + v.y, excl + v.x + v.y + v.z);
        if (t == 255u)
        {
            block_offset[SORT_SCAN_BLOCKS + blockIdx.x] = excl + sum;
            __threadfence();
            is_last = atomicAdd(done_counter, 1u) == gridDim.x - 1u;
        }
        __syncthreads();
        if (is_last && t < 32u)
        {
            __threadfence();
            constexpr uint32_t PER_LANE = SORT_SCAN_BLOCKS / 32;
            uint32_t lane_sum = 0;
            for (uint32_t k = 0; k < PER_LANE; k++) lane_sum += block_offset[SORT_SCAN_BLOCKS + t * PER_LANE + k];
            uint32_t inc = lane_sum;
            for (int off = 1; off < 32; off <<= 1)
            {
                const uint32_t u = __shfl_up_sync(0xFFFFFFFFu, inc, off);
                if (t >= (uint32_t)off) inc += u;
            }
            uint32_t run = inc - lane_sum;
            for (uint32_t k = 0; k < PER_LANE; k++)
            {
                const uint32_t tot = block_offset[SORT_SCAN_BLOCKS + t * PER_LANE + k];
                block_offset[t * PER_LANE + k] = run;
                run += tot;
            }
            if (t == 0) *done_counter = 0u;
        }
    }

    static __global__ void __launch_bounds__(256) k_sort_scatter(const uint32_t* key, const uint32_t* rank, const uint32_t* bin_start,
                                                                 const uint32_t* block_offset, uint32_t* order, const uint32_t* n_ptr)
    {
        const uint32_t n = *n_ptr;
        for (uint32_t i = blockIdx.x * blockDim.x + threadIdx.x; i < n; i += gridDim.x * blockDim.x)
        {
            const uint32_t k = key[i];
            order[block_offset[k >> 10] + bin_start[k] + rank[i]] = i;
        }
    }

    template <uint32_t FEATS, class R>
    MCRT_D void queryInteraction(const WaveParams<R>& p, const KnnQuery<R>& qr, Interaction<R>& ia)
    {
        ia.type = IA_DIFFUSE;
        ia.n1 = qr.pos_n1.w; ia.n2 = qr.nrm_n2.w; ia.Rf = qr.out_rf.w; ia.T = qr.weight_t.w;
        ia.material = &p.scene.materials[qr.meta.x];
        ia.fmask = FEATS;
        ia.out = qr.out_rf.xyz();
        ia.shading_cs = Frame<R>(qr.nrm_n2.xyz());
        ia.inside = qr.meta.z & 1u;
    }

    template <class R>
    MCRT_D bool photonTerm(Interaction<R>& ia, uint32_t which, const float4& a, const float4& b, R d2, R inv_r2, V3<R>& term)
    {
        V3<R> bsdf_absIdotN; R bsdf_pdf;
        if (!ia.bsdfWorld(bsdf_absIdotN, photonDir<R>(b.z, b.w), bsdf_pdf)) return false;
        const V3<R> flux((R)a.x, (R)a.y, (R)a.z);
        if (which == 0)
        {
            const R wp = gmax(R(0), R(1) - msqrt(d2 * inv_r2));
            term = (flux * bsdf_absIdotN * wp) / bsdf_pdf;
        }
        else
        {
            term = flux * bsdf_absIdotN / bsdf_pdf;
        }
        return true;
    }

    template <class R, class Scale>
    MCRT_D void depositGroupRuns(const WaveParams<R>& p, uint32_t film_index, uint32_t plane, const V3<R>& sum, const V3<R>& weight,
                                 Scale&& scale)
    {
        const unsigned lane = threadIdx.x & 31u;
        unsigned pending = __ballot_sync(0xFFFFFFFFu, plane != NO_PRIM);
        while (pending)
        {
            const int leader = __ffs(pending) - 1;
            const uint32_t g = __shfl_sync(0xFFFFFFFFu, plane, leader);
            const bool mine = plane == g;
            V3<R> v = mine ? sum : V3<R>(R(0));
            for (int off = 16; off > 0; off >>= 1)
            {
                v.x += __shfl_xor_sync(0xFFFFFFFFu, v.x, off);
                v.y += __shfl_xor_sync(0xFFFFFFFFu, v.y, off);
                v.z += __shfl_xor_sync(0xFFFFFFFFu, v.z, off);
            }
            if ((int)lane == leader) filmAddV(p.film + g * p.plane_values, film_index, scale(v) * weight);
            pending &= ~__ballot_sync(0xFFFFFFFFu, mine);
        }
    }

    template <class R, class Scale>
    MCRT_D void groupRunStep(const WaveParams<R>& p, uint32_t film_index, const V3<R>& weight, Scale&& scale, uint32_t g,
                             const V3<R>& term, uint32_t& run, V3<R>& run_sum)
    {
        const bool flush = g != NO_PRIM && run != NO_PRIM && g != run;
        if (__any_sync(0xFFFFFFFFu, flush))
        {
            depositGroupRuns(p, film_index, flush ? run : NO_PRIM, run_sum, weight, scale);
            if (flush) { run = NO_PRIM; run_sum = V3<R>(R(0)); }
        }
        if (g != NO_PRIM) { run = g; run_sum += term; }
    }

    template <class R, class Scale>
    MCRT_D void depositMaskRuns(const WaveParams<R>& p, uint32_t film_index, bool has, uint32_t mask, const V3<R>& sum,
                                const V3<R>& weight, Scale&& scale)
    {
        const unsigned lane = threadIdx.x & 31u;
        unsigned pending = __ballot_sync(0xFFFFFFFFu, has);
        while (pending)
        {
            const int leader = __ffs(pending) - 1;
            const uint32_t g = __shfl_sync(0xFFFFFFFFu, mask, leader);
            const bool mine = has && mask == g;
            V3<R> v = mine ? sum : V3<R>(R(0));
            for (int off = 16; off > 0; off >>= 1)
            {
// ... 247 lines not shown
                           V3<R> bsdf_absIdotN; R bsdf_pdf;
                           if (ia.bsdfWorld(bsdf_absIdotN, photonDir<R>(b.z, b.w), bsdf_pdf))
                           {
                               const V3<R> flux((R)a.x, (R)a.y, (R)a.z);
                               if (which == 0)
                               {
                                   const R wp = gmax(R(0), R(1) - msqrt((R)d2 * inv_r2));
                                   sum += (flux * bsdf_absIdotN * wp) / bsdf_pdf;
                               }
                               else
                               {
                                   sum += flux * bsdf_absIdotN / bsdf_pdf;
                               }
                           }
                       });
            if (!__any_sync(0xFFFFFFFFu, found)) continue;
            for (int off = 16; off > 0; off >>= 1)
            {
                sum.x += __shfl_xor_sync(0xFFFFFFFFu, sum.x, off);
                sum.y += __shfl_xor_sync(0xFFFFFFFFu, sum.y, off);
                sum.z += __shfl_xor_sync(0xFFFFFFFFu, sum.z, off);
            }
            if (lane == 0)
            {
                V3<R> radiance = which == 0 ? R(3) * sum * inv_r2 * Consts<R>::INV_PI : sum / ((R)r2 * Consts<R>::PI);
                depositRadiance<FILM>(p, qr.meta.y, pixelOfFilmIndex(p, qr.meta.y), qr.meta.w, radiance * qr.weight_t.xyz(), NO_PRIM,
                                      MCRT_PM_CAUSTIC + which);
            }
            __syncwarp();
        }
        if (lane == 0 && overflow) atomicOr(&p.counters->traversal_overflow, 1u);
        if (threadIdx.x == 0 && blockIdx.x == 0) atomicAdd(&p.counters->knn_queries, (unsigned long long)n);
    }


    template <class R, bool LPE>
    __global__ void __launch_bounds__(256) k_emit_generate(WaveParams<R> p, int next)
    {
        Counters* c = p.counters;
        const uint32_t n_next = c->n_next;
        const unsigned long long remaining = c->total_work - c->next_work;
        const uint32_t room = p.capacity - n_next;
        const uint32_t count = remaining < (unsigned long long)room ? (uint32_t)remaining : room;
        if (blockIdx.x == 0 && threadIdx.x == 0) c->n_gen = count;
        const unsigned long long base_work = c->next_work;
        const PathBuffer<R>& out = p.buf[next];
        const DeviceScene<R>& sc = p.scene;

        const uint32_t count_rounded = (count + 31u) & ~31u;
        for (uint32_t j = blockIdx.x * blockDim.x + threadIdx.x; j < count_rounded; j += gridDim.x * blockDim.x)
        {
            const bool valid = j < count;
            uint32_t key = 0;
            const uint32_t slot = n_next + j;
            if (valid)
            {
                const unsigned long long w = base_work + j;
                uint32_t lo = 0, hi = sc.n_lights;
                while (hi - lo > 1) { const uint32_t mid = (lo + hi) / 2; if (p.emit.emit_offsets[mid] <= w) lo = mid; else hi = mid; }
                const uint32_t light = lo;
                const unsigned long long n_light = p.emit.emit_offsets[light + 1] - p.emit.emit_offsets[light];
                const uint32_t index = (uint32_t)((unsigned long long)p.emit.pass * n_light + (w - p.emit.emit_offsets[light]));
                SamplerState smp = SamplerState::make(p.global_seed, light, index, 0u);
                R u[4];
                samplerGet<R, DIM_PM_LIGHT, 4>(smp, u);
                V3<R> pos, normal;
                sampleLightPoint(sc.lights[light], u[0], u[1], pos, normal);
                const V3<R> dir = Frame<R>(normal).from(cosWeightedHemi(u[2], u[3]));
                pos += normal * p.ray_eps;
                const V4<R> flux = p.emit.photon_flux[light];
                out.ray_o[slot] = V4<R>(pos, sc.scene_ior);
                out.ray_d[slot] = V4<R>(dir, R(1));
                out.thr[slot] = V4<R>(flux.x, flux.y, flux.z, R(0));
                out.meta[slot] = make_uint4(light, index, 0u, 0u);
                uint32_t lpe_state = 0;
                if constexpr (LPE)
                    lpe_state = p.emit.lpe_rev_start == MCRT_LPE_DEAD ? (uint32_t)MCRT_LPE_DEAD
                              : (uint32_t)__ldg(&p.emit.lpe_rev_next[p.emit.lpe_rev_start * p.lpe_symbols + lpeLightSymbol(p, light)]);
                out.meta2[slot] = make_uint4(NO_PRIM, 1u | (lpe_state << 16), 0u, sc.lights[light].type == PRIM_TRIANGLE ? sc.lights[light].prim : NO_PRIM);
                if (p.sort.path_order) key = rayKey(p.sort, pos, dir, sc.lights[light].prim);
            }
            if (p.sort.path_order)
            {
                const uint32_t rank = sortRank(p.sort.hist_path, key, valid);
                if (valid) { p.sort.path_key[next][slot] = key; p.sort.path_rank[next][slot] = rank; }
            }
        }
    }

    MCRT_D void storePhoton(float4* arr, unsigned long long idx, const V3<double>& flux, const V3<double>& pos, const V3<double>& dir)
    {
        const float theta = (float)atan2(sqrt(dir.x * dir.x + dir.y * dir.y), dir.z);
        const float phi = (float)atan2(dir.y, dir.x);
        arr[2 * idx] = make_float4((float)flux.x, (float)flux.y, (float)flux.z, (float)pos.x);
        arr[2 * idx + 1] = make_float4((float)pos.y, (float)pos.z, phi, theta);
    }

    template <class R, bool LPE>
    __global__ void __launch_bounds__(128, MCRT_SHADE_MINBLOCKS) k_emit_shade(WaveParams<R> p, int cur)
    {
        __shared__ SobolByteTables sobol_tab;
        sobol_tab.fill(p.sobol_bytes);
        __syncthreads();
        Counters* c = p.counters;
        const uint32_t n = c->n_cur;
        const PathBuffer<R>& in = p.buf[cur];
        const PathBuffer<R>& out = p.buf[cur ^ 1];
        const DeviceScene<R>& sc = p.scene;
        const bool sorting = p.sort.path_order != nullptr;
        uint32_t local_max_depth = 0, stack_overflows = 0;

        const uint32_t n_rounded = (n + 31u) & ~31u;
        for (uint32_t i = blockIdx.x * blockDim.x + threadIdx.x; i < n_rounded; i += gridDim.x * blockDim.x)
        {
            bool alive = i < n;
            int store = -1;
            V3<R> ph_flux, ph_pos, ph_dir;
            PathRay<R> ray, nray;
            V3<R> flux;
            uint4 meta, meta2;
            uint32_t ior_count = 1, hit_prim = NO_PRIM;
            R iors[IOR_STACK_CAPACITY];
            uint32_t lpe_state = 0, lpe_next = 0;

            if (alive)
            {
                const V4<R> ro = ldStream(&in.ray_o[i]), rd = ldStream(&in.ray_d[i]), th = ldStream(&in.thr[i]), hv = ldStream(&p.hits[i]);
                meta = ldStream(&in.meta[i]); meta2 = ldStream(&in.meta2[i]);
                if constexpr (LPE) lpe_state = (meta2.y >> 16) & 0xFFu;
                ray.start = ro.xyz(); ray.medium_ior = ro.w;
                ray.direction = rd.xyz(); ray.refraction_scale = rd.w;
                flux = th.xyz();
                ray.depth = meta.z & 0xFFFFu; ray.diffuse_depth = meta.z >> 16;
                ray.refraction_level = (int32_t)meta.w;
                ior_count = meta2.y & 0xFFu;
                ray.dirac_delta = (meta2.y >> 8) & 1u;
                ray.refraction = false;
                iors[0] = sc.scene_ior;
                if (ior_count > 1)
                {
                    const V4<R> ia_ = in.iors_a[i];
                    iors[1] = ia_.x; iors[2] = ia_.y; iors[3] = ia_.z; iors[4] = ia_.w;
                    if (ior_count > 5) { const V4<R> ib_ = in.iors_b[i]; iors[5] = ib_.x; iors[6] = ib_.y; iors[7] = ib_.z; }
                }
                if (ray.depth > local_max_depth) local_max_depth = ray.depth;

                Hit<R> hit;
                hit.t = hv.x; hit.u = hv.y; hit.v = hv.z;
                hit.prim = hv.w < R(0) ? NO_PRIM : (uint32_t)hv.w;
                hit_prim = hit.prim;
                if (hit.prim == NO_PRIM)
                {
                    alive = false;
                }
                else
                {
                    SamplerState smp = SamplerState::make(p.global_seed, meta.x, meta.y, ray.depth + 1u);
                    smp.tab = &sobol_tab;
                    int ext_idx = ray.refraction_level - 1;
                    ext_idx = ext_idx < 0 ? 0 : (ext_idx > (int)ior_count - 1 ? (int)ior_count - 1 : ext_idx);
                    Interaction<R> ia;
                    buildInteraction(ia, sc, hit, ray, iors[ext_idx], smp);
                    const Material<R>& m = *ia.material;
                    if constexpr (LPE)
                        lpe_next = lpe_state == MCRT_LPE_DEAD ? (uint32_t)MCRT_LPE_DEAD
                                 : (uint32_t)__ldg(&p.emit.lpe_rev_next[lpe_state * p.lpe_symbols + lpeVertexSymbol(ia.type, ia.dirac_delta)]);

                    if (!(m.flags & MAT_DIRAC_DELTA))
                    {
                        if (ray.dirac_delta)
                        {
                            store = 0; ph_flux = flux;
                        }
                        else
                        {
                            R ur;
                            samplerGet<R, DIM_PM_REJECT, 1>(smp, &ur);
                            if (p.emit.non_caustic_reject > ur) { store = 1; ph_flux = flux / p.emit.non_caustic_reject; }
                        }
                        ph_pos = ia.position; ph_dir = -ray.direction;
                    }

                    V3<R> bsdf_absIdotN; R bsdf_pdf;
                    if (!sampleBSDF(ia, ray, smp, p.ray_eps, true, bsdf_absIdotN, bsdf_pdf, nray))
                    {
                        alive = false;
                    }
                    else
                    {
                        bsdf_absIdotN /= bsdf_pdf;
                        R survive = gmin(compMax(bsdf_absIdotN), R(0.95));
                        R ua;
                        samplerGet<R, DIM_ABSORB, 1>(smp, &ua);
                        if (survive == R(0) || survive <= ua) alive = false;
                        else
                        {
                            flux *= bsdf_absIdotN / survive;
                            if (nray.refraction_level > 0)
                            {
                                if (nray.refraction_level == (int32_t)ior_count)
                                {
                                    if (ior_count < (uint32_t)IOR_STACK_CAPACITY) iors[ior_count++] = nray.medium_ior;
                                    else stack_overflows++;
                                }
                                else if (nray.refraction_level < (int32_t)ior_count - 1) ior_count--;
                            }
                        }
                    }
                }
            }

            for (int which = 0; which < 2; which++)
            {
                const bool mine = store == which;
                const unsigned mask = __ballot_sync(0xFFFFFFFFu, mine);
                if (mask)
                {
                    const unsigned lane = threadIdx.x & 31u;
                    const int leader = __ffs(mask) - 1;
                    unsigned long long base = 0;
                    if ((int)lane == leader) base = atomicAdd(&c->n_photons[which], (unsigned long long)__popc(mask));
                    base = __shfl_sync(0xFFFFFFFFu, base, leader);
                    if (mine)
                    {
                        const unsigned long long idx = base + __popc(mask & ((1u << lane) - 1u));
                        if (idx < p.emit.capacity[which])
                        {
                            storePhoton(p.emit.photons[which], idx, V3<double>((double)ph_flux.x, (double)ph_flux.y, (double)ph_flux.z),
                                        V3<double>((double)ph_pos.x, (double)ph_pos.y, (double)ph_pos.z),
                                        V3<double>((double)ph_dir.x, (double)ph_dir.y, (double)ph_dir.z));
                            p.emit.lights[which][idx] = meta.x;
                            if constexpr (LPE) p.emit.lpe_states[which][idx] = lpe_state;
                        }
                        else c->photon_overflow = 1u;
                    }
                }
            }

            const uint32_t slot = warpAppend(&c->n_next, alive);
            uint32_t pkey = 0, prank = 0;
            if (sorting && alive)
            {
                pkey = rayKey(p.sort, nray.start, nray.direction, hit_prim);
                prank = atomicAdd(&p.sort.hist_path[pkey], 1u);
            }
            if (alive)
            {
                out.ray_o[slot] = V4<R>(nray.start, nray.medium_ior);
                out.ray_d[slot] = V4<R>(nray.direction, nray.refraction_scale);
                out.thr[slot] = V4<R>(flux, R(0));
                if (ior_count > 1)
                {
                    out.iors_a[slot] = V4<R>(iors[1], iors[2], iors[3], iors[4]);
                    if (ior_count > 5) out.iors_b[slot] = V4<R>(iors[5], iors[6], iors[7], R(0));
                }
                out.meta[slot] = make_uint4(meta.x, meta.y, (nray.depth & 0xFFFFu) | (nray.diffuse_depth << 16), (uint32_t)nray.refraction_level);
                out.meta2[slot] = make_uint4(NO_PRIM, ior_count | (nray.dirac_delta ? 256u : 0u) | (lpe_next << 16), 0u,
                                             sc.shade[hit_prim].type == PRIM_TRIANGLE ? hit_prim : NO_PRIM);
                if (sorting) { p.sort.path_key[cur ^ 1][slot] = pkey; p.sort.path_rank[cur ^ 1][slot] = prank; }
            }
        }
        if (local_max_depth) atomicMax(&c->max_depth, local_max_depth);
        if (stack_overflows) atomicAdd(&c->ior_stack_overflows, (unsigned long long)stack_overflows);
    }

    template <class R, bool FAST>
    __global__ void __launch_bounds__(256) k_trace_user(DeviceScene<R> sc, const double* rays6, size_t n, double* out_tuv,
                                                        uint32_t* out_prim, Counters* c)
    {
        TraceCounters cnt = { 0u, 0u, 0u };
        uint32_t overflow = 0;
        unsigned long long rays = 0;
        for (size_t i = blockIdx.x * (size_t)blockDim.x + threadIdx.x; i < n; i += (size_t)gridDim.x * blockDim.x)
        {
            const double* r = rays6 + 6 * i;
            Hit<R> h = traceClosest<PRIMS_ALL, FAST>(sc, V3<R>((R)r[0], (R)r[1], (R)r[2]), V3<R>((R)r[3], (R)r[4], (R)r[5]), NO_PRIM, cnt, overflow);
            out_tuv[3 * i + 0] = (double)h.t; out_tuv[3 * i + 1] = (double)h.u; out_tuv[3 * i + 2] = (double)h.v;
            out_prim[i] = h.prim;
            rays++;
        }
        flushStats(c, cnt, rays, false, overflow);
    }

    template <class R, bool FAST>
    __global__ void __launch_bounds__(256) k_features(DeviceScene<R> sc, DeviceCamera<R> cam, uint32_t global_seed,
                                                      uint32_t sample_first, uint32_t sample_count, double* out, Counters* c)
    {
        TraceCounters cnt = { 0u, 0u, 0u };
        uint32_t overflow = 0;
        unsigned long long rays = 0;
        const uint32_t n = cam.width * cam.height;
        for (uint32_t pixel = blockIdx.x * blockDim.x + threadIdx.x; pixel < n; pixel += gridDim.x * blockDim.x)
        {
            double* f = out + 8 * (size_t)pixel;
            double sum[8];
            for (int k = 0; k < 8; k++) sum[k] = f[k];
            for (uint32_t k = 0; k < sample_count; k++)
            {
                const SamplerState smp = SamplerState::make(global_seed, pixel, sample_first + k, 0u);
                V3<R> start, direction;
                cameraRay(cam, sc.scene_ior, pixel, smp, start, direction);
                const Hit<R> h = traceClosest<PRIMS_ALL, FAST>(sc, start, direction, NO_PRIM, cnt, overflow);
                rays++;
                if (h.prim == NO_PRIM) continue;
                const PrimShade<R> ps = sc.shade[h.prim];
                const Material<R>& m = sc.materials[ps.material];
                const V3<R> albedo = (m.flags & (MAT_PERFECT_MIRROR | MAT_COMPLEX_IOR)) ? m.specular_reflectance : m.reflectance;
                V3<R> normal, shading_normal;
                surfaceNormals(sc, ps, h, start + direction * h.t, direction, normal, shading_normal);
                sum[0] += (double)albedo.x; sum[1] += (double)albedo.y; sum[2] += (double)albedo.z;
                sum[3] += (double)shading_normal.x; sum[4] += (double)shading_normal.y; sum[5] += (double)shading_normal.z;
                sum[6] += (double)h.t;
                sum[7] += 1.0;
            }
            for (int k = 0; k < 8; k++) f[k] = sum[k];
        }
        flushStats(c, cnt, rays, false, overflow);
    }


    template <class R, bool FAST>
    __global__ void __launch_bounds__(256) k_features_chain(DeviceScene<R> sc, DeviceCamera<R> cam, uint32_t global_seed,
                                                            uint32_t sample_first, uint32_t sample_count, uint32_t specular_depth,
                                                            R ray_eps, double* out, Counters* c)
    {
        TraceCounters cnt = { 0u, 0u, 0u };
        uint32_t overflow = 0;
        unsigned long long rays = 0;
        const uint32_t n = cam.width * cam.height;
        for (uint32_t pixel = blockIdx.x * blockDim.x + threadIdx.x; pixel < n; pixel += gridDim.x * blockDim.x)
        {
            double* f = out + 8 * (size_t)pixel;
            double sum[8];
            for (int k = 0; k < 8; k++) sum[k] = f[k];
            for (uint32_t k = 0; k < sample_count; k++)
            {
                const uint32_t sample = sample_first + k;
                PathRay<R> ray;
                cameraRay(cam, sc.scene_ior, pixel, SamplerState::make(global_seed, pixel, sample, 0u), ray.start, ray.direction);
                ray.medium_ior = sc.scene_ior; ray.refraction_scale = R(1);
                ray.depth = 0u; ray.diffuse_depth = 0u; ray.refraction_level = 0;
                ray.dirac_delta = false; ray.refraction = false;
// ... 137 lines not shown
```

### monte-carlo-ray-tracer_b200/csrc/kernels_f64.cu

```cuda
#define MCRT_REAL double
#include "kernels_impl.cuh"

namespace mcrt
{
    void launchAdvance(Counters* c, cudaStream_t s) { k_advance<<<1, 1, 0, s>>>(c); }

    void launchSortScan(uint32_t* hist, const RaySort& rs, cudaStream_t s)
    {
        k_sort_scan<<<SORT_SCAN_BLOCKS, 256, 0, s>>>(hist, rs.bin_start, rs.block_offset, rs.done_counter);
    }

    void launchSortScatter(const uint32_t* key, const uint32_t* rank, const RaySort& rs, uint32_t* order,
                           const uint32_t* n_ptr, int grid, cudaStream_t s)
    {
        k_sort_scatter<<<grid, 256, 0, s>>>(key, rank, rs.bin_start, rs.block_offset, order, n_ptr);
    }

    void launchResolveFilmWeighted(const double* film, const double* wsum, double* out, size_t n_pixels, int grid, cudaStream_t s)
    {
        k_resolve_film_weighted<<<grid, 256, 0, s>>>(film, wsum, out, n_pixels);
    }

    void launchResolveFilm(const double* film, double* out, size_t n_values, double weight, int grid, cudaStream_t s)
    {
        k_resolve_film<<<grid, 256, 0, s>>>(film, out, n_values, weight);
    }

    void launchResolveFilmPeers(const double* film, const PeerFrames& pf, size_t n_values, double weight, int grid, cudaStream_t s)
    {
        k_resolve_film_peers<<<grid, 256, 0, s>>>(film, pf, n_values, weight);
    }

    template <bool TILE_COUNTS>
    static __global__ void __launch_bounds__(256) k_progressive_resolve(ProgressiveHalf a, ProgressiveHalf b, uint32_t weighted,
                                                                        uint32_t width, uint32_t rows, uint32_t tile,
                                                                        uint32_t tiles_x, uint32_t n_tiles, double* out, double* sums,
                                                                        const double* tile_counts)
    {
        const uint64_t n = (uint64_t)width * rows;
        const bool both = a.samples > 0.0 && b.samples > 0.0;
        const double scale = both ? a.samples * b.samples / ((a.samples + b.samples) * (a.samples + b.samples)) : 0.0;
        const unsigned lane = threadIdx.x & 31u;
        const uint64_t n_rounded = (n + 31u) & ~31ull;
        for (uint64_t i = blockIdx.x * (uint64_t)blockDim.x + threadIdx.x; i < n_rounded; i += (uint64_t)gridDim.x * blockDim.x)
        {
            double v = 0.0, i2 = 0.0;
            uint32_t key = 0xFFFFFFFFu;
            if (i < n)
            {
                double na = a.samples, nb = b.samples, pixel_scale = scale;
                bool pixel_both = both;
                if constexpr (TILE_COUNTS)
                {
                    const uint32_t y = (uint32_t)(i / width), x = (uint32_t)(i - (uint64_t)y * width);
                    const size_t t = (size_t)(y / tile) * tiles_x + x / tile;
                    na = tile_counts[2 * t]; nb = tile_counts[2 * t + 1];
                    pixel_both = na > 0.0 && nb > 0.0;
                    pixel_scale = pixel_both ? na * nb / ((na + nb) * (na + nb)) : 0.0;
                }
                const double wa = !a.rgb ? 0.0 : (weighted ? a.wsum[i] : na);
                const double wb = !b.rgb ? 0.0 : (weighted ? b.wsum[i] : nb);
                const double w = wa + wb;
                const bool compare = pixel_both && wa != 0.0 && wb != 0.0;
                for (int c = 0; c < 3; c++)
                {
                    const double sa = a.rgb ? a.rgb[3 * i + c] : 0.0, sb = b.rgb ? b.rgb[3 * i + c] : 0.0;
                    double value = w == 0.0 ? 0.0 : (sa + sb) / w;
                    value = value < 0.0 ? 0.0 : value;
                    out[3 * i + c] = value;
                    i2 += value * value;
                    if (compare)
                    {
                        const double d = sa / wa - sb / wb;
                        v += d * d * pixel_scale;
                    }
                }
                const uint32_t y = (uint32_t)(i / width), x = (uint32_t)(i - (uint64_t)y * width);
                key = (y / tile) * tiles_x + x / tile;
            }
            double fv = v, fi = i2;
            for (int off = 16; off > 0; off >>= 1)
            {
                fv += __shfl_xor_sync(0xFFFFFFFFu, fv, off);
                fi += __shfl_xor_sync(0xFFFFFFFFu, fi, off);
            }
            if (lane == 0)
            {
                if (fv != 0.0) atomicAdd(&sums[2 * (size_t)n_tiles], fv);
                if (fi != 0.0) atomicAdd(&sums[2 * (size_t)n_tiles + 1], fi);
            }
            unsigned pending = __ballot_sync(0xFFFFFFFFu, key != 0xFFFFFFFFu);
            while (pending)
            {
                const int leader = __ffs(pending) - 1;
                const uint32_t k = __shfl_sync(0xFFFFFFFFu, key, leader);
                const bool mine = key == k;
                double gv = mine ? v : 0.0, gi = mine ? i2 : 0.0;
                for (int off = 16; off > 0; off >>= 1)
// ... 156 lines not shown
```

### monte-carlo-ray-tracer_b200/csrc/launch.h

```cpp
#pragma once

#include "integrator.cuh"

namespace mcrt
{
    template <class R> struct Launch
    {
        static void generate(const WaveParams<R>& p, int next, int grid, cudaStream_t s);
        static void extend(const WaveParams<R>& p, int cur, int grid, cudaStream_t s);
        static void shade(const WaveParams<R>& p, int cur, int grid, cudaStream_t s);
        static void shadePhoton(const WaveParams<R>& p, int cur, int grid, cudaStream_t s);
        static void knn(const WaveParams<R>& p, int grid, cudaStream_t s);
        static void emitGenerate(const WaveParams<R>& p, int next, int grid, cudaStream_t s);
        static void emitShade(const WaveParams<R>& p, int cur, int grid, cudaStream_t s);
        static void shadow(const WaveParams<R>& p, int grid, cudaStream_t s);
        static void shadeKey(const WaveParams<R>& p, int grid, cudaStream_t s);
        static void traceUser(const DeviceScene<R>& sc, const double* rays6, size_t n, double* out_tuv,
                              uint32_t* out_prim, Counters* c, int grid, cudaStream_t s);
        static void features(const DeviceScene<R>& sc, const DeviceCamera<R>& cam, uint32_t global_seed, uint32_t sample_first,
                             uint32_t sample_count, double* out, Counters* c, int grid, cudaStream_t s);
        static void featuresChain(const DeviceScene<R>& sc, const DeviceCamera<R>& cam, uint32_t global_seed, uint32_t sample_first,
                                  uint32_t sample_count, uint32_t specular_depth, R ray_eps, double* out, Counters* c, int grid,
                                  cudaStream_t s);
    };

    void launchAdvance(Counters* c, cudaStream_t s);
    void launchSortScan(uint32_t* hist, const RaySort& rs, cudaStream_t s);
    void launchSortScatter(const uint32_t* key, const uint32_t* rank, const RaySort& rs, uint32_t* order,
                           const uint32_t* n_ptr, int grid, cudaStream_t s);
    void launchResolveFilmWeighted(const double* film, const double* wsum, double* out, size_t n_pixels, int grid, cudaStream_t s);
    void launchResolveFilm(const double* film, double* out, size_t n_values, double weight, int grid, cudaStream_t s);
    void launchResolveFilmPeers(const double* film, const PeerFrames& pf, size_t n_values, double weight, int grid, cudaStream_t s);
    void launchProgressiveResolve(const ProgressiveHalf& a, const ProgressiveHalf& b, bool weighted, uint32_t width, uint32_t rows,
                                  uint32_t tile, uint32_t tiles_x, double* out, double* sums, double* tile_error, uint32_t n_tiles,
                                  int grid, cudaStream_t s, const double* tile_counts = nullptr);
    void launchLightGroupsCombine(const double* planes, uint32_t n_planes, uint64_t n_values, const double* weights, double* out,
                                  int grid, cudaStream_t s);
    void launchFp64Peak(double* sink, int iterations, int grid, cudaStream_t s);
    void launchKnnUser(const DevicePhotonMap& map, uint32_t k, const double* points, size_t n, uint32_t* out_index,
                       double* out_d2, uint32_t* out_count, uint32_t* overflow_flag, int grid, cudaStream_t s);
    void launchGatherUser(const DevicePhotonMap& map, const double* points, size_t n, double r2, uint32_t* out_count,
                          double* out_flux, double* out_cone, uint32_t* overflow_flag, int grid, cudaStream_t s);
    void launchSamplerStream(const uint32_t* pixel, const uint32_t* sample, size_t n, uint32_t n_shuffles,
                             uint32_t global_seed, uint32_t* out, cudaStream_t s);
}
```

Measured before the change: 2844.

## Replace atomic-rank ray sort scatter with two-pass coarse/fine tiled counting sort

Result: faster. 2880 (median of 6 runs) (+1.3%).

```diff
diff --git a/include/mcrt_abi.h b/include/mcrt_abi.h
--- a/include/mcrt_abi.h
+++ b/include/mcrt_abi.h
@@ -363,6 +363,8 @@
 int mcrt_sampler_stream(mcrt_ctx* ctx, const uint32_t* pixel, const uint32_t* sample, size_t n,
                         uint32_t n_shuffles, uint32_t global_seed, uint32_t* out_u32x7);
 
+int mcrt_sort_keys(mcrt_ctx* ctx, const uint32_t* keys, size_t n, uint32_t* out_order);
+
 int mcrt_knn_search(mcrt_ctx* ctx, int which, const double* points_xyz, size_t n,
                     uint32_t* out_index, double* out_dist2, uint32_t* out_count,
                     mcrt_stats* stats);
diff --git a/monte-carlo-ray-tracer_b200/__init__.py b/monte-carlo-ray-tracer_b200/__init__.py
--- a/monte-carlo-ray-tracer_b200/__init__.py
+++ b/monte-carlo-ray-tracer_b200/__init__.py
@@ -18,7 +18,7 @@
     "mcrt_photon_upload", "mcrt_photon_emit", "mcrt_photon_download", "mcrt_octree_build",
     "mcrt_octree_free", "mcrt_render_rows", "mcrt_render_rows_dev", "mcrt_render_rows_strided_dev",
     "mcrt_trace_closest",
-    "mcrt_sample_rays", "mcrt_sampler_stream", "mcrt_knn_search", "mcrt_set_option", "mcrt_set_film",
+    "mcrt_sample_rays", "mcrt_sampler_stream", "mcrt_sort_keys", "mcrt_knn_search", "mcrt_set_option", "mcrt_set_film",
     "mcrt_obj_load", "mcrt_obj_free", "mcrt_obj_vertex_normals",
     "mcrt_bvh_build", "mcrt_bvh_free", "mcrt_image_tonemap", "mcrt_image_tonemap_dev",
     "mcrt_render_rows_strided_peers", "mcrt_frame_alloc", "mcrt_frame_open", "mcrt_frame_close", "mcrt_frame_free",
@@ -276,6 +276,7 @@
         L.mcrt_sample_rays.argtypes = [C.c_void_p, C.c_void_p, C.c_void_p, C.c_void_p, C.c_size_t, C.c_uint32,
                                        C.c_int, C.c_int, C.c_void_p, C.POINTER(Stats)]
         L.mcrt_sampler_stream.argtypes = [C.c_void_p, C.c_void_p, C.c_void_p, C.c_size_t, C.c_uint32, C.c_uint32, C.c_void_p]
+        L.mcrt_sort_keys.argtypes = [C.c_void_p, C.c_void_p, C.c_size_t, C.c_void_p]
         L.mcrt_knn_search.argtypes = [C.c_void_p, C.c_int, C.c_void_p, C.c_size_t, C.c_void_p, C.c_void_p,
                                       C.c_void_p, C.POINTER(Stats)]
         L.mcrt_set_option.argtypes = [C.c_void_p, C.c_char_p, C.c_double]
@@ -800,6 +801,12 @@
         out = np.zeros((len(pixel), 7), dtype=np.uint32)
         self._check(lib().mcrt_sampler_stream(self.ctx, _ptr(pixel), _ptr(sample), len(pixel), n_shuffles,
                                               self.global_seed, _ptr(out)))
+        return out
+
+    def sort_keys(self, keys):
+        keys = np.ascontiguousarray(keys, dtype=np.uint32)
+        out = np.zeros(len(keys), dtype=np.uint32)
+        self._check(lib().mcrt_sort_keys(self.ctx, _ptr(keys), len(keys), _ptr(out)))
         return out
 
 
diff --git a/monte-carlo-ray-tracer_b200/csrc/abi.cu b/monte-carlo-ray-tracer_b200/csrc/abi.cu
--- a/monte-carlo-ray-tracer_b200/csrc/abi.cu
+++ b/monte-carlo-ray-tracer_b200/csrc/abi.cu
@@ -578,16 +578,11 @@
         int rc;
         RaySort& r = ctx->sort;
         for (int b = 0; b < 2; b++)
-        {
             if ((rc = devAlloc(ctx, ctx->sort_allocs, &r.path_key[b], n))) return rc;
-            if ((rc = devAlloc(ctx, ctx->sort_allocs, &r.path_rank[b], n))) return rc;
-        }
         if ((rc = devAlloc(ctx, ctx->sort_allocs, &r.path_order, n))) return rc;
         if ((rc = devAlloc(ctx, ctx->sort_allocs, &r.shadow_key, n))) return rc;
-        if ((rc = devAlloc(ctx, ctx->sort_allocs, &r.shadow_rank, n))) return rc;
         if ((rc = devAlloc(ctx, ctx->sort_allocs, &r.shadow_order, n))) return rc;
         if ((rc = devAlloc(ctx, ctx->sort_allocs, &r.shade_key, n))) return rc;
-        if ((rc = devAlloc(ctx, ctx->sort_allocs, &r.shade_rank, n))) return rc;
         if ((rc = devAlloc(ctx, ctx->sort_allocs, &r.shade_order, n))) return rc;
         if ((rc = devAlloc(ctx, ctx->sort_allocs, &r.hist_shade, (size_t)SORT_BINS))) return rc;
         if ((rc = devAlloc(ctx, ctx->sort_allocs, &r.hist_path, (size_t)SORT_BINS))) return rc;
@@ -595,6 +590,11 @@
         if ((rc = devAlloc(ctx, ctx->sort_allocs, &r.bin_start, (size_t)SORT_BINS))) return rc;
         if ((rc = devAlloc(ctx, ctx->sort_allocs, &r.block_offset, (size_t)2 * SORT_SCAN_BLOCKS))) return rc;
         if ((rc = devAlloc(ctx, ctx->sort_allocs, &r.done_counter, (size_t)1))) return rc;
+        if ((rc = devAlloc(ctx, ctx->sort_allocs, &r.coarse_start, (size_t)SORT_COARSE + 1))) return rc;
+        if ((rc = devAlloc(ctx, ctx->sort_allocs, &r.coarse_cursor, (size_t)SORT_COARSE))) return rc;
+        if ((rc = devAlloc(ctx, ctx->sort_allocs, &r.chunk_start, (size_t)SORT_COARSE + 1))) return rc;
+        if ((rc = devAlloc(ctx, ctx->sort_allocs, &r.part_slot, n))) return rc;
+        if ((rc = devAlloc(ctx, ctx->sort_allocs, &r.part_fine, n))) return rc;
         CK(cudaMemset(r.done_counter, 0, sizeof(uint32_t)));
         ctx->sort_capacity = ctx->pool_paths;
         return MCRT_OK;
@@ -844,9 +844,7 @@
         }
         auto sortPaths = [&](int buffer)
         {
-            launchSortScan(p.sort.hist_path, p.sort, s);
-            launchSortScatter(p.sort.path_key[buffer], p.sort.path_rank[buffer], p.sort, p.sort.path_order,
-                              &ctx->d_counters->n_cur, grid, s);
+            launchSortQueue(p.sort.path_key[buffer], p.sort.hist_path, p.sort, p.sort.path_order, &ctx->d_counters->n_cur, grid, s);
         };
 
         uint64_t launches = 0, iterations = 0;
@@ -855,7 +853,7 @@
         else Launch<R>::generate(p, 0, grid, s);
         launchAdvance(ctx->d_counters, s);
         launches += 2;
-        if (sorting) { sortPaths(0); launches += 2; }
+        if (sorting) { sortPaths(0); launches += 3; }
 
         int pending[2] = { 0, 0 };
         int slot = 0;
@@ -882,9 +880,8 @@
                 if (p.sort.shade_order)
                 {
                     Launch<R>::shadeKey(p, grid, s);
-                    launchSortScan(p.sort.hist_shade, p.sort, s);
-                    launchSortScatter(p.sort.shade_key, p.sort.shade_rank, p.sort, p.sort.shade_order, &ctx->d_counters->n_cur, grid, s);
-                    launches += 3;
+                    launchSortQueue(p.sort.shade_key, p.sort.hist_shade, p.sort, p.sort.shade_order, &ctx->d_counters->n_cur, grid, s);
+                    launches += 4;
                 }
                 if (emitting)
                 {
@@ -906,10 +903,9 @@
                 {
                     if (sorting)
                     {
-                        launchSortScan(p.sort.hist_shadow, p.sort, s);
-                        launchSortScatter(p.sort.shadow_key, p.sort.shadow_rank, p.sort, p.sort.shadow_order,
-                                          &ctx->d_counters->n_shadow, grid, s);
-                        launches += 2;
+                        launchSortQueue(p.sort.shadow_key, p.sort.hist_shadow, p.sort, p.sort.shadow_order,
+                                        &ctx->d_counters->n_shadow, grid, s);
+                        launches += 3;
                     }
                     Launch<R>::shadow(p, grid, s);
                 }
@@ -917,7 +913,7 @@
                 if (emitting) Launch<R>::emitGenerate(p, cur ^ 1, grid, s);
                 else Launch<R>::generate(p, cur ^ 1, grid, s);
                 launchAdvance(ctx->d_counters, s);
-                if (sorting) { sortPaths(cur ^ 1); launches += 2; }
+                if (sorting) { sortPaths(cur ^ 1); launches += 3; }
                 if (ev) cudaEventRecord(ev[4], s);
                 launches += 5;
                 iterations++;
@@ -2725,6 +2721,33 @@
     return MCRT_OK;
 }
 
+int mcrt_sort_keys(mcrt_ctx* ctx, const uint32_t* keys, size_t n, uint32_t* out_order)
+{
+    if (!ctx) return MCRT_ERR_INVALID;
+    if (n && (!keys || !out_order)) { ctx->error = "mcrt_sort_keys: null buffer"; return MCRT_ERR_INVALID; }
+    if (n > ctx->pool_paths) { ctx->error = "mcrt_sort_keys: more keys than the path pool holds"; return MCRT_ERR_INVALID; }
+    std::vector<uint32_t> hist(SORT_BINS, 0u);
+    for (size_t i = 0; i < n; i++)
+    {
+        if (keys[i] >= SORT_BINS) { ctx->error = "mcrt_sort_keys: key outside the ray-sort key range"; return MCRT_ERR_INVALID; }
+        hist[keys[i]]++;
+    }
+    CK(cudaSetDevice(ctx->device));
+    int rc;
+    if ((rc = ensureSort(ctx))) return rc;
+    cudaStream_t s = ctx->stream;
+    const uint32_t n32 = (uint32_t)n;
+    CK(cudaMemcpyAsync(ctx->sort.shade_key, keys, n * 4, cudaMemcpyHostToDevice, s));
+    CK(cudaMemcpyAsync(ctx->sort.hist_shade, hist.data(), SORT_BINS * 4, cudaMemcpyHostToDevice, s));
+    CK(cudaMemcpyAsync(&ctx->d_counters->n_cur, &n32, 4, cudaMemcpyHostToDevice, s));
+    launchSortQueue(ctx->sort.shade_key, ctx->sort.hist_shade, ctx->sort, ctx->sort.shade_order, &ctx->d_counters->n_cur,
+                    ctx->sm_count * ctx->blocks_per_sm, s);
+    CK(cudaMemcpyAsync(out_order, ctx->sort.shade_order, n * 4, cudaMemcpyDeviceToHost, s));
+    CK(cudaStreamSynchronize(s));
+    CK(cudaGetLastError());
+    return MCRT_OK;
+}
+
 int mcrt_knn_search(mcrt_ctx* ctx, int which, const double* points_xyz, size_t n, uint32_t* out_index, double* out_dist2,
                     uint32_t* out_count, mcrt_stats* stats)
 {
diff --git a/monte-carlo-ray-tracer_b200/csrc/integrator.cuh b/monte-carlo-ray-tracer_b200/csrc/integrator.cuh
--- a/monte-carlo-ray-tracer_b200/csrc/integrator.cuh
+++ b/monte-carlo-ray-tracer_b200/csrc/integrator.cuh
@@ -37,6 +37,9 @@
 #ifndef MCRT_SORT_ORIGIN_BITS
 #define MCRT_SORT_ORIGIN_BITS 4
 #endif
+#ifndef MCRT_SORT_COARSE_BITS
+#define MCRT_SORT_COARSE_BITS 8
+#endif
 #ifndef MCRT_SORT_DIR_Q
 #define MCRT_SORT_DIR_Q 1
 #endif
@@ -87,23 +90,36 @@
     constexpr uint32_t SORT_DIR_BITS = 3 + 2 * SORT_DIR_Q;
     constexpr uint32_t SORT_KEY_BITS = 3 * SORT_ORIGIN_BITS + SORT_DIR_BITS;
     constexpr uint32_t SORT_BINS = 1u << SORT_KEY_BITS;
+    constexpr uint32_t SORT_COARSE_BITS = MCRT_SORT_COARSE_BITS;
+    constexpr uint32_t SORT_FINE_BITS = SORT_KEY_BITS - SORT_COARSE_BITS;
+    constexpr uint32_t SORT_COARSE = 1u << SORT_COARSE_BITS;
+    constexpr uint32_t SORT_FINE = 1u << SORT_FINE_BITS;
+    constexpr uint32_t SORT_THREADS = 256;
+    constexpr uint32_t SORT_ITEMS = 16;
+    constexpr uint32_t SORT_CHUNK = SORT_THREADS * SORT_ITEMS;
+    static_assert(SORT_FINE_BITS <= 16 && SORT_COARSE <= SORT_THREADS && SORT_COARSE % 32 == 0,
+                  "fine digits are stored in 16 bits; one thread per coarse digit");
+    static_assert(SORT_FINE % SORT_THREADS == 0, "k_sort_fine scans SORT_FINE / SORT_THREADS digits per thread");
+    static_assert(SORT_CHUNK == 4096 && SORT_KEY_BITS <= 20, "k_sort_partition packs key << 12 | position in the tile in 32 bits");
 
     struct RaySort
     {
         uint32_t* path_key[2];
-        uint32_t* path_rank[2];
         uint32_t* path_order;
         uint32_t* shadow_key;
-        uint32_t* shadow_rank;
         uint32_t* shadow_order;
         uint32_t* hist_path;
         uint32_t* hist_shadow;
         uint32_t* bin_start;
         uint32_t* block_offset;
         uint32_t* done_counter;
+        uint32_t* coarse_start;
+        uint32_t* coarse_cursor;
+        uint32_t* chunk_start;
+        uint32_t* part_slot;
+        uint16_t* part_fine;
         uint32_t shade_sorted;
         uint32_t* shade_key;
-        uint32_t* shade_rank;
         uint32_t* shade_order;
         uint32_t* hist_shade;
         uint32_t prim_scale;
@@ -152,21 +168,32 @@
         return (dir << (3 * SORT_ORIGIN_BITS)) | cell;
     }
 
-    MCRT_D uint32_t sortRank(uint32_t* hist, uint32_t key, bool pred)
+    MCRT_D void sortCount(uint32_t* hist, uint32_t key, bool pred)
     {
         const unsigned active = __ballot_sync(0xFFFFFFFFu, pred);
-        uint32_t rank = 0;
         if (pred)
         {
             const unsigned peers = __match_any_sync(active, key);
-            const unsigned lane = threadIdx.x & 31u;
-            const int leader = __ffs(peers) - 1;
-            uint32_t base = 0;
-            if ((int)lane == leader) base = atomicAdd(&hist[key], (uint32_t)__popc(peers));
-            base = __shfl_sync(peers, base, leader);
-            rank = base + __popc(peers & ((1u << lane) - 1u));
-        }
-        return rank;
+            if ((int)(threadIdx.x & 31u) == __ffs(peers) - 1) atomicAdd(&hist[key], (uint32_t)__popc(peers));
+        }
+    }
+
+    template <uint32_t BITS>
+    MCRT_D uint32_t digitRank(uint32_t* s_hist, uint32_t digit, bool pred)
+    {
+        unsigned peers = __ballot_sync(0xFFFFFFFFu, pred);
+#pragma unroll
+        for (uint32_t b = 0; b < BITS; b++)
+        {
+            const unsigned ones = __ballot_sync(0xFFFFFFFFu, (digit >> b) & 1u);
+            peers &= ((digit >> b) & 1u) ? ones : ~ones;
+        }
+        const unsigned lane = threadIdx.x & 31u;
+        const int leader = pred ? __ffs(peers) - 1 : (int)lane;
+        uint32_t base = 0;
+        if (pred && (int)lane == leader) base = atomicAdd(&s_hist[digit], (uint32_t)__popc(peers));
+        base = __shfl_sync(0xFFFFFFFFu, base, leader);
+        return base + __popc(peers & ((1u << lane) - 1u));
     }
 
     template <class R> struct EmitParams
@@ -477,8 +504,8 @@
             }
             if (p.sort.path_order)
             {
-                const uint32_t rank = sortRank(p.sort.hist_path, key, valid);
-                if (valid) { p.sort.path_key[next][slot] = key; p.sort.path_rank[next][slot] = rank; }
+                sortCount(p.sort.hist_path, key, valid);
+                if (valid) p.sort.path_key[next][slot] = key;
             }
         }
     }
@@ -864,16 +891,16 @@
 
             const uint32_t slot = warpAppend(&c->n_next, alive);
             const uint32_t sslot = warpAppend(&c->n_shadow, want_shadow);
-            uint32_t pkey = 0, prank = 0, skey = 0, srank = 0;
+            uint32_t pkey = 0, skey = 0;
             if (sorting && alive)
             {
                 pkey = rayKey(p.sort, nray.start, nray.direction, hit_prim);
-                prank = atomicAdd(&p.sort.hist_path[pkey], 1u);
+                atomicAdd(&p.sort.hist_path[pkey], 1u);
             }
             if (sorting && want_shadow)
             {
                 skey = rayKey(p.sort, sh_o, sh_d, hit_prim);
-                srank = atomicAdd(&p.sort.hist_shadow[skey], 1u);
+                atomicAdd(&p.sort.hist_shadow[skey], 1u);
             }
             if (alive)
             {
@@ -890,7 +917,7 @@
                 stStream(&out.meta2[slot], make_uint4(ls_light, ior_count | (nray.dirac_delta ? 256u : 0u) | (lobe << 9) |
                                                                     (FILM == FILM_MODE_LPE ? lpe_state << 16 : 0u), meta2.z,
                                                       sc.shade[hit_prim].type == PRIM_TRIANGLE ? hit_prim : NO_PRIM));
-                if (sorting) { p.sort.path_key[cur ^ 1][slot] = pkey; p.sort.path_rank[cur ^ 1][slot] = prank; }
+                if (sorting) p.sort.path_key[cur ^ 1][slot] = pkey;
             }
             if (want_shadow)
             {
@@ -901,7 +928,7 @@
                                                 FILM == FILM_MODE_AOV || FILM == FILM_MODE_LPE ? sh_plane : meta.y));
                 if constexpr (sizeof(R) == 8) stStream(reinterpret_cast<uint4*>(&srec) + 5, make_uint4(0u, 0u, 0u, 0u));
                 stStream(&srec.k, V4<R>(sh_k, sh_select));
-                if (sorting) { p.sort.shadow_key[sslot] = skey; p.sort.shadow_rank[sslot] = srank; }
+                if (sorting) p.sort.shadow_key[sslot] = skey;
             }
 
             if constexpr (KIND == 1)
@@ -983,11 +1010,12 @@
 
 
     constexpr uint32_t SHADE_CLASS_BINS = 64;
+    static_assert(SHADE_CLASS_BINS <= SORT_FINE, "the classes are keys of sortQueue's first bucket");
 
     template <class R>
     __global__ void __launch_bounds__(256) k_shade_key(WaveParams<R> p)
     {
-        __shared__ uint32_t s_hist[SHADE_CLASS_BINS], s_base[SHADE_CLASS_BINS];
+        __shared__ uint32_t s_hist[SHADE_CLASS_BINS];
         const uint32_t n = p.counters->n_cur;
         const uint32_t chunks = (n + 255u) / 256u;
         for (uint32_t chunk = blockIdx.x; chunk < chunks; chunk += gridDim.x)
@@ -995,28 +1023,27 @@
             if (threadIdx.x < SHADE_CLASS_BINS) s_hist[threadIdx.x] = 0u;
             __syncthreads();
             const uint32_t i = chunk * 256u + threadIdx.x;
-            uint32_t key = 0, local = 0;
             if (i < n)
             {
                 const R w = p.hits[i].w;
-                if (!(w < R(0))) key = p.scene.shade_class[(uint32_t)w];
-                local = atomicAdd(&s_hist[key], 1u);
+                const uint32_t key = w < R(0) ? 0u : p.scene.shade_class[(uint32_t)w];
+                atomicAdd(&s_hist[key], 1u);
+                p.sort.shade_key[i] = key;
             }
             __syncthreads();
-            if (threadIdx.x < SHADE_CLASS_BINS && s_hist[threadIdx.x]) s_base[threadIdx.x] = atomicAdd(&p.sort.hist_shade[threadIdx.x], s_hist[threadIdx.x]);
+            if (threadIdx.x < SHADE_CLASS_BINS && s_hist[threadIdx.x]) atomicAdd(&p.sort.hist_shade[threadIdx.x], s_hist[threadIdx.x]);
             __syncthreads();
-            if (i < n) { p.sort.shade_key[i] = key; p.sort.shade_rank[i] = s_base[key] + local; }
-            __syncthreads();
         }
     }
 
     constexpr uint32_t SORT_SCAN_BLOCKS = SORT_BINS / 1024;
 
-    static __global__ void __launch_bounds__(256) k_sort_scan(uint32_t* hist, uint32_t* bin_start, uint32_t* block_offset,
-                                                              uint32_t* done_counter)
+    static __global__ void __launch_bounds__(256) k_sort_scan(uint32_t* hist, RaySort rs)
     {
         __shared__ uint32_t warp_sums[8];
         __shared__ uint32_t is_last;
+        uint32_t* bin_start = rs.bin_start;
+        uint32_t* block_offset = rs.block_offset;
         const uint32_t t = threadIdx.x, base = blockIdx.x * 1024u + t * 4u;
         const uint4 v = *reinterpret_cast<const uint4*>(hist + base);
         *reinterpret_cast<uint4*>(hist + base) = make_uint4(0u, 0u, 0u, 0u);
@@ -1033,19 +1060,17 @@
         for (uint32_t w = 0; w < (t >> 5); w++) warp_base += warp_sums[w];
         const uint32_t excl = warp_base + incl - sum;
         *reinterpret_cast<uint4*>(bin_start + base) = make_uint4(excl, excl + v.x, excl + v.x + v.y, excl + v.x + v.y + v.z);
-        if (t == 255u)
-        {
-            block_offset[SORT_SCAN_BLOCKS + blockIdx.x] = excl + sum;
-            __threadfence();
-            is_last = atomicAdd(done_counter, 1u) == gridDim.x - 1u;
-        }
+        if (t == 255u) block_offset[SORT_SCAN_BLOCKS + blockIdx.x] = excl + sum;
+        __threadfence();
+        __syncthreads();
+        if (t == 255u) is_last = atomicAdd(rs.done_counter, 1u) == gridDim.x - 1u;
         __syncthreads();
         if (is_last && t < 32u)
         {
             __threadfence();
             constexpr uint32_t PER_LANE = SORT_SCAN_BLOCKS / 32;
             uint32_t lane_sum = 0;
-            for (uint32_t k = 0; k < PER_LANE; k++) lane_sum += block_offset[SORT_SCAN_BLOCKS + t * PER_LANE + k];
+            for (uint32_t k = 0; k < PER_LANE; k++) lane_sum += __ldcg(&block_offset[SORT_SCAN_BLOCKS + t * PER_LANE + k]);
             uint32_t inc = lane_sum;
             for (int off = 1; off < 32; off <<= 1)
             {
@@ -1055,22 +1080,174 @@
             uint32_t run = inc - lane_sum;
             for (uint32_t k = 0; k < PER_LANE; k++)
             {
-                const uint32_t tot = block_offset[SORT_SCAN_BLOCKS + t * PER_LANE + k];
+                const uint32_t tot = __ldcg(&block_offset[SORT_SCAN_BLOCKS + t * PER_LANE + k]);
                 block_offset[t * PER_LANE + k] = run;
                 run += tot;
             }
-            if (t == 0) *done_counter = 0u;
-        }
-    }
-
-    static __global__ void __launch_bounds__(256) k_sort_scatter(const uint32_t* key, const uint32_t* rank, const uint32_t* bin_start,
-                                                                 const uint32_t* block_offset, uint32_t* order, const uint32_t* n_ptr)
-    {
+            const uint32_t total = __shfl_sync(0xFFFFFFFFu, run, 31);
+            __syncwarp();
+            constexpr uint32_t B_LANE = SORT_COARSE / 32;
+            uint32_t start[B_LANE + 1];
+            for (uint32_t k = 0; k <= B_LANE; k++)
+            {
+                const uint32_t b = t * B_LANE + k;
+                const uint32_t key = b << SORT_FINE_BITS;
+                start[k] = b < SORT_COARSE ? __ldcg(&block_offset[key >> 10]) + __ldcg(&bin_start[key]) : total;
+            }
+            uint32_t chunks = 0;
+            for (uint32_t k = 0; k < B_LANE; k++) chunks += (start[k + 1] - start[k] + SORT_CHUNK - 1) / SORT_CHUNK;
+            uint32_t cinc = chunks;
+            for (int off = 1; off < 32; off <<= 1)
+            {
+                const uint32_t u = __shfl_up_sync(0xFFFFFFFFu, cinc, off);
+                if (t >= (uint32_t)off) cinc += u;
+            }
+            uint32_t chunk = cinc - chunks;
+            for (uint32_t k = 0; k < B_LANE; k++)
+            {
+                const uint32_t b = t * B_LANE + k;
+                rs.coarse_start[b] = start[k];
+                rs.coarse_cursor[b] = start[k];
+                rs.chunk_start[b] = chunk;
+                chunk += (start[k + 1] - start[k] + SORT_CHUNK - 1) / SORT_CHUNK;
+            }
+            if (t == 31u)
+            {
+                rs.coarse_start[SORT_COARSE] = total;
+                rs.chunk_start[SORT_COARSE] = chunk;
+                *rs.done_counter = 0u;
+            }
+        }
+    }
+
+    static __global__ void __launch_bounds__(SORT_THREADS) k_sort_partition(const uint32_t* key, const uint32_t* n_ptr, RaySort rs)
+    {
+        __shared__ uint32_t s_count[SORT_COARSE], s_local[SORT_COARSE], s_base[SORT_COARSE];
+        __shared__ uint32_t s_key[SORT_CHUNK];
+        __shared__ uint32_t s_warp[SORT_THREADS / 32];
         const uint32_t n = *n_ptr;
-        for (uint32_t i = blockIdx.x * blockDim.x + threadIdx.x; i < n; i += gridDim.x * blockDim.x)
-        {
-            const uint32_t k = key[i];
-            order[block_offset[k >> 10] + bin_start[k] + rank[i]] = i;
+        const uint32_t tiles = (n + SORT_CHUNK - 1) / SORT_CHUNK;
+        for (uint32_t tile = blockIdx.x; tile < tiles; tile += gridDim.x)
+        {
+            if (threadIdx.x < SORT_COARSE) s_count[threadIdx.x] = 0u;
+            __syncthreads();
+            const uint32_t first = tile * SORT_CHUNK, m = min(SORT_CHUNK, n - first);
+            uint32_t k[SORT_ITEMS], rank[SORT_ITEMS];
+#pragma unroll
+            for (uint32_t q = 0; q < SORT_ITEMS; q++)
+            {
+                const uint32_t e = q * SORT_THREADS + threadIdx.x;
+                k[q] = e < m ? __ldcs(key + first + e) : 0u;
+            }
+#pragma unroll
+            for (uint32_t q = 0; q < SORT_ITEMS; q++)
+                rank[q] = digitRank<SORT_COARSE_BITS>(s_count, k[q] >> SORT_FINE_BITS, q * SORT_THREADS + threadIdx.x < m);
+            __syncthreads();
+            const uint32_t c = threadIdx.x < SORT_COARSE ? s_count[threadIdx.x] : 0u;
+            uint32_t incl = c;
+            for (int off = 1; off < 32; off <<= 1)
+            {
+                const uint32_t u = __shfl_up_sync(0xFFFFFFFFu, incl, off);
+                if ((threadIdx.x & 31u) >= (uint32_t)off) incl += u;
+            }
+            if ((threadIdx.x & 31u) == 31u) s_warp[threadIdx.x >> 5] = incl;
+            __syncthreads();
+            if (threadIdx.x < SORT_COARSE)
+            {
+                uint32_t run = incl - c;
+                for (uint32_t w = 0; w < (threadIdx.x >> 5); w++) run += s_warp[w];
+                s_local[threadIdx.x] = run;
+                s_base[threadIdx.x] = c ? atomicAdd(&rs.coarse_cursor[threadIdx.x], c) : 0u;
+            }
+            __syncthreads();
+#pragma unroll
+            for (uint32_t q = 0; q < SORT_ITEMS; q++)
+            {
+                const uint32_t e = q * SORT_THREADS + threadIdx.x;
+                if (e < m) s_key[s_local[k[q] >> SORT_FINE_BITS] + rank[q]] = (k[q] << 12) | e;
+            }
+            __syncthreads();
+            for (uint32_t e = threadIdx.x; e < m; e += SORT_THREADS)
+            {
+                const uint32_t v = s_key[e], kk = v >> 12, b = kk >> SORT_FINE_BITS;
+                const uint32_t pos = s_base[b] + e - s_local[b];
+                rs.part_slot[pos] = first + (v & (SORT_CHUNK - 1u));
+                rs.part_fine[pos] = (uint16_t)(kk & (SORT_FINE - 1u));
+            }
+            __syncthreads();
+        }
+    }
+
+    static __global__ void __launch_bounds__(SORT_THREADS) k_sort_fine(RaySort rs, uint32_t* order)
+    {
+        constexpr uint32_t PER = (SORT_FINE + SORT_THREADS - 1) / SORT_THREADS;
+        __shared__ uint32_t s_count[SORT_FINE], s_local[SORT_FINE], s_base[SORT_FINE];
+        __shared__ uint32_t s_slot[SORT_CHUNK];
+        __shared__ uint16_t s_fine[SORT_CHUNK];
+        __shared__ uint32_t s_warp[SORT_THREADS / 32];
+        const uint32_t chunks = rs.chunk_start[SORT_COARSE];
+        for (uint32_t j = blockIdx.x; j < chunks; j += gridDim.x)
+        {
+            uint32_t b = 0, b_end = SORT_COARSE;
+            while (b_end - b > 1u)
+            {
+                const uint32_t mid = (b + b_end) / 2u;
+                if (rs.chunk_start[mid] <= j) b = mid; else b_end = mid;
+            }
+            const uint32_t first = rs.coarse_start[b] + (j - rs.chunk_start[b]) * SORT_CHUNK;
+            const uint32_t m = min(SORT_CHUNK, rs.coarse_start[b + 1] - first);
+            for (uint32_t f = threadIdx.x; f < SORT_FINE; f += SORT_THREADS) s_count[f] = 0u;
+            __syncthreads();
+            uint32_t slot[SORT_ITEMS], fine_rank[SORT_ITEMS];
+#pragma unroll
+            for (uint32_t q = 0; q < SORT_ITEMS; q++)
+            {
+                const uint32_t e = q * SORT_THREADS + threadIdx.x;
+                slot[q] = e < m ? __ldcs(rs.part_slot + first + e) : 0u;
+                fine_rank[q] = e < m ? (uint32_t)__ldcs(rs.part_fine + first + e) : 0u;
+            }
+#pragma unroll
+            for (uint32_t q = 0; q < SORT_ITEMS; q++)
+                fine_rank[q] |= digitRank<SORT_FINE_BITS>(s_count, fine_rank[q], q * SORT_THREADS + threadIdx.x < m) << 16;
+            __syncthreads();
+            uint32_t sum = 0;
+            for (uint32_t q = 0; q < PER; q++) sum += s_count[threadIdx.x * PER + q];
+            uint32_t incl = sum;
+            for (int off = 1; off < 32; off <<= 1)
+            {
+                const uint32_t u = __shfl_up_sync(0xFFFFFFFFu, incl, off);
+                if ((threadIdx.x & 31u) >= (uint32_t)off) incl += u;
+            }
+            if ((threadIdx.x & 31u) == 31u) s_warp[threadIdx.x >> 5] = incl;
+            __syncthreads();
+            uint32_t run = incl - sum;
+            for (uint32_t w = 0; w < (threadIdx.x >> 5); w++) run += s_warp[w];
+            for (uint32_t q = 0; q < PER; q++)
+            {
+                const uint32_t f = threadIdx.x * PER + q, key = (b << SORT_FINE_BITS) | f;
+                const uint32_t c = s_count[f];
+                s_local[f] = run;
+                s_base[f] = c ? rs.block_offset[key >> 10] + atomicAdd(&rs.bin_start[key], c) : 0u;
+                run += c;
+            }
+            __syncthreads();
+#pragma unroll
+            for (uint32_t q = 0; q < SORT_ITEMS; q++)
+            {
+                if (q * SORT_THREADS + threadIdx.x < m)
+                {
+                    const uint32_t f = fine_rank[q] & 0xFFFFu, e = s_local[f] + (fine_rank[q] >> 16);
+                    s_slot[e] = slot[q];
+                    s_fine[e] = (uint16_t)f;
+                }
+            }
+            __syncthreads();
+            for (uint32_t e = threadIdx.x; e < m; e += SORT_THREADS)
+            {
+                const uint32_t f = s_fine[e];
+                order[s_base[f] + e - s_local[f]] = s_slot[e];
+            }
+            __syncthreads();
         }
     }
 
@@ -1484,8 +1661,8 @@
             }
             if (p.sort.path_order)
             {
-                const uint32_t rank = sortRank(p.sort.hist_path, key, valid);
-                if (valid) { p.sort.path_key[next][slot] = key; p.sort.path_rank[next][slot] = rank; }
+                sortCount(p.sort.hist_path, key, valid);
+                if (valid) p.sort.path_key[next][slot] = key;
             }
         }
     }
@@ -1640,11 +1817,11 @@
             }
 
             const uint32_t slot = warpAppend(&c->n_next, alive);
-            uint32_t pkey = 0, prank = 0;
+            uint32_t pkey = 0;
             if (sorting && alive)
             {
                 pkey = rayKey(p.sort, nray.start, nray.direction, hit_prim);
-                prank = atomicAdd(&p.sort.hist_path[pkey], 1u);
+                atomicAdd(&p.sort.hist_path[pkey], 1u);
             }
             if (alive)
             {
@@ -1659,7 +1836,7 @@
                 out.meta[slot] = make_uint4(meta.x, meta.y, (nray.depth & 0xFFFFu) | (nray.diffuse_depth << 16), (uint32_t)nray.refraction_level);
                 out.meta2[slot] = make_uint4(NO_PRIM, ior_count | (nray.dirac_delta ? 256u : 0u) | (lpe_next << 16), 0u,
                                              sc.shade[hit_prim].type == PRIM_TRIANGLE ? hit_prim : NO_PRIM);
-                if (sorting) { p.sort.path_key[cur ^ 1][slot] = pkey; p.sort.path_rank[cur ^ 1][slot] = prank; }
+                if (sorting) p.sort.path_key[cur ^ 1][slot] = pkey;
             }
         }
         if (local_max_depth) atomicMax(&c->max_depth, local_max_depth);
diff --git a/monte-carlo-ray-tracer_b200/csrc/kernels_f64.cu b/monte-carlo-ray-tracer_b200/csrc/kernels_f64.cu
--- a/monte-carlo-ray-tracer_b200/csrc/kernels_f64.cu
+++ b/monte-carlo-ray-tracer_b200/csrc/kernels_f64.cu
@@ -5,15 +5,12 @@
 {
     void launchAdvance(Counters* c, cudaStream_t s) { k_advance<<<1, 1, 0, s>>>(c); }
 
-    void launchSortScan(uint32_t* hist, const RaySort& rs, cudaStream_t s)
-    {
-        k_sort_scan<<<SORT_SCAN_BLOCKS, 256, 0, s>>>(hist, rs.bin_start, rs.block_offset, rs.done_counter);
-    }
-
-    void launchSortScatter(const uint32_t* key, const uint32_t* rank, const RaySort& rs, uint32_t* order,
-                           const uint32_t* n_ptr, int grid, cudaStream_t s)
-    {
-        k_sort_scatter<<<grid, 256, 0, s>>>(key, rank, rs.bin_start, rs.block_offset, order, n_ptr);
+    void launchSortQueue(const uint32_t* key, uint32_t* hist, const RaySort& rs, uint32_t* order, const uint32_t* n_ptr, int grid,
+                         cudaStream_t s)
+    {
+        k_sort_scan<<<SORT_SCAN_BLOCKS, 256, 0, s>>>(hist, rs);
+        k_sort_partition<<<grid, SORT_THREADS, 0, s>>>(key, n_ptr, rs);
+        k_sort_fine<<<grid, SORT_THREADS, 0, s>>>(rs, order);
     }
 
     void launchResolveFilmWeighted(const double* film, const double* wsum, double* out, size_t n_pixels, int grid, cudaStream_t s)
diff --git a/monte-carlo-ray-tracer_b200/csrc/launch.h b/monte-carlo-ray-tracer_b200/csrc/launch.h
--- a/monte-carlo-ray-tracer_b200/csrc/launch.h
+++ b/monte-carlo-ray-tracer_b200/csrc/launch.h
@@ -25,9 +25,8 @@
     };
 
     void launchAdvance(Counters* c, cudaStream_t s);
-    void launchSortScan(uint32_t* hist, const RaySort& rs, cudaStream_t s);
-    void launchSortScatter(const uint32_t* key, const uint32_t* rank, const RaySort& rs, uint32_t* order,
-                           const uint32_t* n_ptr, int grid, cudaStream_t s);
+    void launchSortQueue(const uint32_t* key, uint32_t* hist, const RaySort& rs, uint32_t* order, const uint32_t* n_ptr, int grid,
+                         cudaStream_t s);
     void launchResolveFilmWeighted(const double* film, const double* wsum, double* out, size_t n_pixels, int grid, cudaStream_t s);
     void launchResolveFilm(const double* film, double* out, size_t n_values, double weight, int grid, cudaStream_t s);
     void launchResolveFilmPeers(const double* film, const PeerFrames& pf, size_t n_values, double weight, int grid, cudaStream_t s);
```
